# sasg/cilium

Hardware: AMD Instinct MI355X
Metric: classified headers/sec (Mpps, whole node) at 100k-prefix ipcache + 16k-ID policy (higher is better)
Workload: dtype u32

## Files before the change

cilium_amd/_lib.py:

```python
import ctypes
import os

HERE = os.path.dirname(os.path.abspath(__file__))
LIB_PATH = os.path.join(HERE, os.environ.get("CFC_LIB", "libcfc.so"))

CFC_DEVICE_NONE = -1
MODE_INGRESS, MODE_EGRESS, MODE_XDP, MODE_FULL = 0, 1, 2, 3
HF_FRAG, HF_TCP_CLOSE, HF_EXTHDR = 0x100, 0x200, 0x400
DROP_PREFILTER, VERDICT_PUNT = -1, -2
OPT_LPM4, OPT_TIMING, OPT_CT_APPLY, OPT_CT_EVICT = 1, 2, 3, 4
CT_APPLY_DEVICE, CT_APPLY_HOST = 0, 1
LPM4_AUTO, LPM4_DIR24_8, LPM4_TRIE = 0, 1, 2

EXPORTS = (
    "cfc_open", "cfc_close", "cfc_abi_version", "cfc_map_open",
    "cfc_drop_notify_v4", "cfc_drop_notify_v6",
    "cfc_map_close", "cfc_map_update", "cfc_map_lookup", "cfc_map_delete",
    "cfc_map_get_next_key", "cfc_num_possible_cpus", "cfc_endpoint_config",
    "cfc_commit", "cfc_classify_v4", "cfc_counters_device",
    "cfc_counters_sync", "cfc_counters_clear", "cfc_counters_export",
    "cfc_counters_import", "cfc_get_stats", "cfc_strerror",
    "cfc_set_option", "cfc_timing_collect", "cfc_classify_v6",
    "cfc_ct_apply_v4", "cfc_ct_apply_v6", "cfc_map_update_batch",
    "cfc_set_node_config", "cfc_get_node_config", "cfc_identity_counters",
    "cfc_set_clock", "cfc_monitor_events_v4", "cfc_monitor_events_v6",
    "cfc_map_dump", "cfc_ct_gc",
    "cfc_proxy_entries_v4", "cfc_proxy_entries_v6",
    "cfc_proxy_apply_v4", "cfc_proxy_apply_v6",
)
CT_NEW, CT_ESTABLISHED, CT_REPLY, CT_RELATED = 0, 1, 2, 3
CT_RES_MASK, CT_DONE, CT_CREATE = 0x3, 0x4, 0x8


class CfcError(OSError):
    pass


GC_REMOVE_EXPIRED, GC_VALID_IPS, GC_MATCH_IPS = 1, 2, 4


class Ip(ctypes.Structure):
    _fields_ = [("family", ctypes.c_uint8), ("pad", ctypes.c_uint8 * 3),
                ("addr", ctypes.c_uint8 * 16)]


class GcFilter(ctypes.Structure):
    _fields_ = [("flags", ctypes.c_uint32), ("time", ctypes.c_uint32),
                ("valid_ips", ctypes.c_void_p), ("n_valid", ctypes.c_uint32),
                ("pad0", ctypes.c_uint32),
                ("match_ips", ctypes.c_void_p), ("n_match", ctypes.c_uint32),
                ("pad1", ctypes.c_uint32)]


class GcStats(ctypes.Structure):
    _fields_ = [("deleted", ctypes.c_uint64), ("alive", ctypes.c_uint64),
                ("device_deleted", ctypes.c_uint64), ("log_deleted", ctypes.c_uint64),
                ("host_deleted", ctypes.c_uint64), ("slots_freed", ctypes.c_uint64)]


_HDR = [("saddr", ctypes.c_void_p), ("daddr", ctypes.c_void_p),
        ("ports", ctypes.c_void_p), ("meta", ctypes.c_void_p),
        ("mark", ctypes.c_void_p), ("tcp_flags", ctypes.c_void_p),
        ("n", ctypes.c_uint64)]


class HdrV4(ctypes.Structure):
    _fields_ = _HDR + [("hash", ctypes.c_void_p)]


class HdrV6(ctypes.Structure):
    _fields_ = _HDR + [("hash", ctypes.c_void_p)]


class Out(ctypes.Structure):
    _fields_ = [("verdict", ctypes.c_void_p), ("identity", ctypes.c_void_p),
                ("action", ctypes.c_void_p), ("ct", ctypes.c_void_p),
                ("notify", ctypes.c_void_p), ("pkt_saddr", ctypes.c_void_p),
                ("pkt_daddr", ctypes.c_void_p), ("pkt_ports", ctypes.c_void_p)]


class Stats(ctypes.Structure):
    _fields_ = [("epoch", ctypes.c_uint64), ("device_bytes", ctypes.c_uint64),
                ("ipcache_v4_prefixes", ctypes.c_uint32),
                ("lpm4_tbl8_groups", ctypes.c_uint32),
                ("policy_entries", ctypes.c_uint32),
                ("endpoints", ctypes.c_uint32),
                ("prefilter_v4_fix", ctypes.c_uint32),
                ("prefilter_v4_dyn", ctypes.c_uint32),
                ("lpm4_layout", ctypes.c_uint32),
                ("lpm4_kib", ctypes.c_uint32),
                ("ipcache_v6_prefixes", ctypes.c_uint32),
                ("lpm6_lengths", ctypes.c_uint32),
                ("lpm6_groups", ctypes.c_uint32),
                ("lpm6_kib", ctypes.c_uint32),
                ("endpoints_v6", ctypes.c_uint32),
                ("prefilter_v6_fix", ctypes.c_uint32),
                ("prefilter_v6_dyn", ctypes.c_uint32),
                ("ct4_entries", ctypes.c_uint32),
                ("ct6_entries", ctypes.c_uint32),
                ("ct_apply_device", ctypes.c_uint32),
                ("ct_apply_host", ctypes.c_uint32),
                ("ct_slots", ctypes.c_uint32),
                ("ct_grown", ctypes.c_uint32),
                ("ct_order_changed", ctypes.c_uint64),
                ("nat_hops", ctypes.c_uint64),
                ("ct_evicted", ctypes.c_uint64),
                ("svc_ordered", ctypes.c_uint64),
                ("ct_apply_sparse", ctypes.c_uint64),
                ("ct_self_segments", ctypes.c_uint64)]


class NodeConfig(ctypes.Structure):
    _fields_ = [("ipv4_cluster_range", ctypes.c_uint32),
                ("ipv4_cluster_mask", ctypes.c_uint32),
                ("router_ip6", ctypes.c_uint8 * 16),
                ("host_ifindex", ctypes.c_uint32)]


class IdentityCount(ctypes.Structure):
    _fields_ = [("identity", ctypes.c_uint32), ("dir", ctypes.c_uint8),
                ("pad", ctypes.c_uint8 * 3),
                ("fwd_packets", ctypes.c_uint64), ("fwd_bytes", ctypes.c_uint64),
                ("drop_packets", ctypes.c_uint64), ("drop_bytes", ctypes.c_uint64)]


IDENTITY_OUT_OF_RANGE = 0xFFFFFFFF


class ProxyStats(ctypes.Structure):
    _fields_ = [("redirects", ctypes.c_uint64), ("entries", ctypes.c_uint64),
                ("created", ctypes.c_uint64), ("updated", ctypes.c_uint64),
                ("failed", ctypes.c_uint64)]


class Timing(ctypes.Structure):
    _fields_ = [("launches", ctypes.c_uint64), ("classify_ms", ctypes.c_double),
                ("count_ms", ctypes.c_double), ("launches_v6", ctypes.c_uint64),
                ("classify_v6_ms", ctypes.c_double), ("count_v6_ms", ctypes.c_double)]


_lib = None


def lib():
    global _lib
    if _lib is not None:
        return _lib
    if not os.path.exists(LIB_PATH):
        raise CfcError(2, f"{LIB_PATH} is not built (run __graft_entry__.build())")
    L = ctypes.CDLL(LIB_PATH)
    vp, u32, u64, i32 = ctypes.c_void_p, ctypes.c_uint32, ctypes.c_uint64, ctypes.c_int
    pint = ctypes.POINTER(ctypes.c_int)
    L.cfc_open.argtypes = [i32, ctypes.POINTER(vp)]
    L.cfc_close.argtypes = [vp]
    L.cfc_close.restype = None
    L.cfc_map_open.argtypes = [vp, ctypes.c_char_p, u32, u32, u32, u32, u32,
                               pint, pint]
    L.cfc_map_close.argtypes = [vp, i32]
    L.cfc_map_update.argtypes = [vp, i32, vp, vp, u64]
    L.cfc_map_lookup.argtypes = [vp, i32, vp, vp]
    L.cfc_map_update_batch.argtypes = [vp, i32, vp, vp, u64, u64]
    L.cfc_map_delete.argtypes = [vp, i32, vp]
    L.cfc_map_get_next_key.argtypes = [vp, i32, vp, vp]
    L.cfc_map_dump.argtypes = [vp, i32, vp, vp, u64, ctypes.POINTER(u64)]
    L.cfc_endpoint_config.argtypes = [vp, ctypes.c_uint16, u32]
    L.cfc_set_node_config.argtypes = [vp, ctypes.POINTER(NodeConfig)]
    L.cfc_get_node_config.argtypes = [vp, ctypes.POINTER(NodeConfig)]
    L.cfc_commit.argtypes = [vp, vp]
    L.cfc_classify_v4.argtypes = [vp, ctypes.POINTER(HdrV4), ctypes.POINTER(Out),
                                  i32, ctypes.c_uint16, vp]
    L.cfc_classify_v6.argtypes = [vp, ctypes.POINTER(HdrV6), ctypes.POINTER(Out),
                                  i32, ctypes.c_uint16, vp]
    L.cfc_ct_apply_v4.argtypes = [vp, ctypes.POINTER(HdrV4), ctypes.POINTER(Out),
                                  i32, ctypes.c_uint16, vp]
    L.cfc_ct_apply_v6.argtypes = [vp, ctypes.POINTER(HdrV6), ctypes.POINTER(Out),
                                  i32, ctypes.c_uint16, vp]
    L.cfc_set_clock.argtypes = [vp, u32]
    L.cfc_ct_gc.argtypes = [vp, i32, ctypes.POINTER(GcFilter), ctypes.POINTER(GcStats), vp]
    for f in (L.cfc_drop_notify_v4, L.cfc_drop_notify_v6,
              L.cfc_monitor_events_v4, L.cfc_monitor_events_v6):
        f.argtypes = [vp, vp, ctypes.POINTER(Out), i32, ctypes.c_uint16, vp, vp,
                      u64, vp, vp]
    for f in (L.cfc_proxy_entries_v4, L.cfc_proxy_entries_v6):
        f.argtypes = [vp, vp, ctypes.POINTER(Out), i32, ctypes.c_uint16, vp, vp,
                      u64, vp, vp]
    for f in (L.cfc_proxy_apply_v4, L.cfc_proxy_apply_v6):
        f.argtypes = [vp, vp, ctypes.POINTER(Out), i32, ctypes.c_uint16,
                      ctypes.POINTER(ProxyStats), vp]
    L.cfc_counters_device.argtypes = [vp, ctypes.POINTER(vp), ctypes.POINTER(u64)]
    L.cfc_counters_sync.argtypes = [vp, vp]
    L.cfc_counters_clear.argtypes = [vp, vp]
    L.cfc_counters_export.argtypes = [vp, vp, u64, vp]
    L.cfc_counters_import.argtypes = [vp, vp, u64, vp]
    L.cfc_get_stats.argtypes = [vp, ctypes.POINTER(Stats)]
    L.cfc_identity_counters.argtypes = [vp, vp, u64, ctypes.POINTER(u64)]
    L.cfc_set_option.argtypes = [vp, i32, ctypes.c_int64]
    L.cfc_timing_collect.argtypes = [vp, ctypes.POINTER(Timing)]
    L.cfc_strerror.argtypes = [i32]
    L.cfc_strerror.restype = ctypes.c_char_p
    _lib = L
    return L


def check(rc, what):
    if rc < 0:
        raise CfcError(-rc, f"{what}: {os.strerror(-rc)}")
    return rc
```

cilium_amd/csrc/cfc_api.cpp:

```cpp
#include <hip/hip_runtime.h>

#include <algorithm>
#include <cerrno>
#include <cstdio>
#include <cstdlib>
#include <cstring>
#include <map>
#include <set>
#include <memory>
#include <mutex>
#include <string>
#include <thread>
#include <unordered_set>
#include <type_traits>
#include <vector>

#include "../../include/cfc.h"
#include "classify.hpp"
#include "selfcut.hpp"
#include "ctmirror.hpp"
#include "flatten.hpp"
#include "maps.hpp"

using namespace cfc;

namespace {

template <class T>
static int upload_vec(DevBuf &b, const std::vector<T> &v, hipStream_t s)
{
    return b.upload(v.data(), v.size() * sizeof(T), s);
}

struct GIpc {
    DevBuf tbl24, tbl8, ovf, l4d, l4c, l4l;
    int layout = 0;
    uint32_t n_prefix4 = 0, tbl8_groups = 0, lpm4_kib = 0;
    uint64_t bytes = 0;
};
struct GIpc6 {
    DevBuf l6[4];
    Lpm6 ipc6{};
    Lpm6Host host;
    uint32_t lpm6_kib = 0, n_prefix6 = 0, lpm6_lengths = 0, lpm6_groups = 0;
    uint64_t bytes = 0;
};
struct GPf {
    DevBuf pf24, pf8, pffix, pfbloom, pf6bloom, l6fix[4], l6dyn[4];
    Lpm6 fix{}, dyn{};
    uint32_t fix_mask = 0, fix_zero = 0, bloom_words = 0, bloom6_words = 0;
    uint32_t n_fix4 = 0, n_dyn4 = 0, n_fix6 = 0, n_dyn6 = 0;
    uint64_t bytes = 0;
};
struct GEp {
    DevBuf lxc4, lxc6, pol, polbloom;
    std::vector<PolSlot> pol_host;
    uint32_t lxc4_mask = 0, lxc6_mask = 0, pol_bloom_words = 0, n_eps = 0, n_eps6 = 0;
    bool lxc4_lds = false, lxc6_lds = false;
    std::unordered_map<int, PolLoc> pol_loc;
    std::vector<std::pair<Map *, std::string>> ctr_owner;
    std::vector<uint32_t> seclabel;
    DevBuf ep_info;
    std::map<uint16_t, uint32_t> nat4;
    DevBuf nat6;
    uint64_t bytes = 0;
};
struct GLb {
    DevBuf lb4, rnat4, lb6, rnat6;
    uint32_t lb4_mask = 0, n_lb4 = 0, lb6_mask = 0, n_lb6 = 0;
    uint64_t bytes = 0;
};
struct GCt {
    CtTab<Ct4Slot> t4;
    CtTab<Ct6Slot> t6;
    DevBuf ct_sum;
    DevBuf ct_st;
    CtMaps ct_maps;
    uint32_t n_nat46 = 0;
    uint64_t bytes = 0;
};
template <bool V6, class G>
auto &tab(G &g)
{
    if constexpr (V6)
        return g.t6;
    else
        return g.t4;
}
template <bool V6>
uint64_t state_base(const GCt &g)
{
    return V6 ? g.t4.slots : 0;
}
struct Epoch {
    uint64_t id = 0;
    std::shared_ptr<GIpc> ipc;
    std::shared_ptr<GIpc6> ipc6;
    std::shared_ptr<GPf> pf;
    std::shared_ptr<GEp> ep;
    std::shared_ptr<GCt> ct;
    std::shared_ptr<GLb> lb;
    DevTables T{};
    cfc_stats st{};
};
struct Retired {
    std::shared_ptr<Epoch> e;
    std::vector<hipEvent_t> ev;
};

}

struct cfc_ctx {
    int device = 0;
    int num_cus = 256;
    std::recursive_mutex mu;
    std::map<std::string, std::unique_ptr<Map>> maps;
    std::map<int, Map *> fds;
    int next_fd = 3;
    std::vector<uint32_t> seclabel = std::vector<uint32_t>(65536, 0);
// ... 47 lines not shown
    DevBuf ord_delbm, ord_mixbm, ord_dfirst, ord_cnt;
    DevBuf ord_ct0;
    DevBuf cta_mon;
    uint64_t n_ord_changed = 0;
    struct NatRec {
        int family = 0;
        const void *saddr = nullptr;
        uint64_t n = 0;
        int mode = 0;
        uint16_t ep = 0;
        uint32_t m = 0;
        hipStream_t stream = nullptr;
        DevBuf idx, rows, outs, ws;
        cfc_hdr_v4 h4{};
        cfc_hdr_v6 h6{};
        cfc_out o{};
    };
    std::map<const void *, NatRec> nat;
    DevBuf nat_list, nat_cnt, nat_tmp;
    DevBuf svo_keys, svo_keys2, svo, svo_cnt, svo_tmp;
    uint64_t n_apply_sparse = 0;
    bool nat46_seen = false, hop_nat46 = false;
    uint64_t n_nat_hops = 0;
    bool ct_evict = true;
    DevBuf evict_bm, evict_maps, evict_rel;
    uint64_t n_evicted = 0;
    uint64_t n_ct_grow = 0;
    DevBuf self_addr, self_rows, self_cnt;
    uint64_t n_self_segs = 0;
    struct SegRec {
        const void *saddr = nullptr;
        uint64_t n = 0, off = 0;
        int mode = 0, family = 0;
        uint16_t ep = 0;
    };
    std::map<const void *, SegRec> segs;
    bool pend = false, pend_v6 = false;
    uint32_t *pend_cnt = nullptr;
    hipEvent_t pend_ev = nullptr;
    DevBuf cta_cxr;

    uint64_t *ctr = nullptr;
    size_t ctr_u64 = 0;
    bool ctr_pending = false;
    hipStream_t last_stream = nullptr;
    hipEvent_t last_done = nullptr;
    uint32_t *ws = nullptr;
    size_t ws_bytes = 0;
    Map *metrics = nullptr;
    std::vector<uint64_t> idc = std::vector<uint64_t>(ID_U64, 0);

    DevBuf nt_ws;
    hipEvent_t nt_done = nullptr;
    hipStream_t nt_stream = nullptr;
    bool nt_pending = false;

    DevBuf px_cnt, px_own, px_last, px_bm, px_blk, px_rec;
    hipEvent_t px_done = nullptr;
    hipStream_t px_stream = nullptr;
    bool px_pending = false;

    bool timing = false;
    std::vector<LaunchTiming> tpool;
    size_t tused = 0;
};

namespace {

void order_after_launches(cfc_ctx *c, hipStream_t s)
{
    if (c->ctr_pending && c->last_done && c->last_stream != s)
        (void)hipStreamWaitEvent(s, c->last_done, 0);
    if (c->nt_pending && c->nt_done && c->nt_stream != s)
        (void)hipStreamWaitEvent(s, c->nt_done, 0);
}

constexpr int NGROUPS = 6;
void group_sigs(cfc_ctx *c, uint64_t sig[NGROUPS])
{
    for (int g = 0; g < NGROUPS; g++)
        sig[g] = 1469598103934665603ull + (uint64_t)g;
    auto mix = [&](int g, uint64_t v) { sig[g] = (sig[g] ^ v) * 1099511628211ull; };
    mix(0, (uint64_t)c->opts.lpm4);
    mix(2, c->seclabel_gen);
    for (auto &kv : c->maps) {
        const Map *m = kv.second.get();
        const uint64_t id = (uint64_t)(uintptr_t)m;
        switch (m->role) {
        case ROLE_IPCACHE:
            mix(0, id); mix(0, m->sgen[0]);
            mix(4, id); mix(4, m->sgen[1]);
            break;
        case ROLE_PF4_FIX: case ROLE_PF4_DYN: case ROLE_PF6_FIX: case ROLE_PF6_DYN:
            mix(1, id); mix(1, m->sgen[0]);
            break;
        case ROLE_LXC:
            mix(2, id); mix(2, m->gen);
            break;
        case ROLE_POLICY:
            mix(2, id); mix(2, m->sgen[0]);
            break;
        case ROLE_CT4: case ROLE_CT6:
            mix(3, id); mix(3, m->sgen[0]);
            mix(2, id);
            break;
        case ROLE_LB4_SVC: case ROLE_LB4_RNAT: case ROLE_LB6_SVC: case ROLE_LB6_RNAT:
            mix(5, id); mix(5, m->gen);
            mix(3, m->kv.empty() ? 0 : 1);
            break;
        default:
            break;
        }
    }
}

void settle(cfc_ctx *c)
{
    if (!c->pend)
        return;
    c->pend = false;
    (void)hipEventSynchronize(c->pend_ev);
    const uint32_t *h = c->pend_cnt;
    cfc_ctx::CtFam &X = c->ctf[c->pend_v6];
    X.claims += h[CTA_CLAIMS];
    X.ins += h[CTA_CLAIMS];
    X.log_used += h[CTA_NLOG];
}

template <class Slot>
int remap_mirror(CtTab<Slot> &T, hipStream_t s)
{
    std::vector<Slot> &h = T.host;
    DevBuf &pend = T.pend;
    if (!pend.p)
        return 0;
    const uint64_t n = h.size();
    std::vector<uint32_t> map(n);
    if (n && (hipMemcpyAsync(map.data(), pend.p, 4 * n, hipMemcpyDeviceToHost, s) != hipSuccess ||
              hipStreamSynchronize(s) != hipSuccess))
        return -EIO;
    std::vector<Slot> nh(T.slots);
    const unsigned nt = std::max(1u, std::min(16u, std::thread::hardware_concurrency()));
    std::vector<uint64_t> tb(nt, 0);
    std::vector<std::thread> th;
    for (unsigned t = 0; t < nt; t++)
        th.emplace_back([&, t]() {
            for (uint64_t i = n * t / nt, e = n * (t + 1) / nt; i < e; i++)
                if (map[i] != 0xFFFFFFFFu) {
                    nh[map[i]] = h[i];
                    tb[t] += h[i].w == CT_TOMBSTONE;
                }
        });
    for (std::thread &x : th)
        x.join();
    uint64_t tt = 0;
    for (uint64_t v : tb)
        tt += v;
    T.tomb = (uint32_t)tt;
    h.swap(nh);
    pend.reset();
    return 0;
}
int mirror_sync(GCt &G, hipStream_t s)
{
    if (int rc = remap_mirror(G.t4, s))
        return rc;
// ... 185 lines not shown
            v[1] += byt;
            if (it == mm->kv.end() && mm->kv.size() >= mm->max_entries)
                continue;
            Map::Entry &e = mm->kv[nk];
            e.key = nk;
            e.val.assign((const char *)v, 16);
            mm->gen++;
        }
    c->ctr_pending = false;
    return 0;
}

int upload_lpm6(DevBuf *b, const Lpm6Host &h, Lpm6 *d, hipStream_t s)
{
    int rc;
    if ((rc = upload_vec(b[0], h.slots, s)) || (rc = upload_vec(b[1], h.bloom, s)) ||
        (rc = upload_vec(b[2], h.lens, s)) || (rc = upload_vec(b[3], h.slots64, s)))
        return rc;
    d->slots = (const L6Slot *)b[0].p;
    d->slots64 = (const uint4 *)b[3].p;
    d->mask64 = h.slots64.empty() ? 0 : (uint32_t)h.slots64.size() - 1;
    d->bloom = (const uint64_t *)b[1].p;
    d->lens = (const uint32_t *)b[2].p;
    d->mask = h.slots.empty() ? 0 : (uint32_t)h.slots.size() - 1;
    d->bloom_mask = h.bloom.empty() ? 0 : (uint32_t)h.bloom.size() - 1;
    d->nlen = (uint32_t)h.lens.size();
    d->def_label = h.def_label;
    return 0;
}

void note_stream(cfc_ctx *c, hipStream_t s)
{
    if (std::find(c->streams.begin(), c->streams.end(), s) == c->streams.end())
        c->streams.push_back(s);
}

uint32_t identity_cover_touched(cfc_ctx *c)
{
    uint32_t cover = 0;
    for (auto &kv : c->maps) {
        Map *m = kv.second.get();
        if (m->role != ROLE_IPCACHE)
            continue;
        for (auto &t : m->touched) {
            auto it = m->kv.find(t.first);
            if (it == m->kv.end())
                continue;
            uint32_t lab;
            memcpy(&lab, it->second.val.data(), 4);
            if (lab < ID_PACK_LIMIT)
                cover |= 1u << id_range_of(lab);
        }
    }
    return cover;
}

void reap_retired(cfc_ctx *c)
{
    auto done = [](const Retired &r) {
        for (hipEvent_t e : r.ev)
            if (hipEventQuery(e) != hipSuccess)
                return false;
        return true;
    };
    for (size_t i = 0; i < c->retired.size();) {
        if (done(c->retired[i])) {
            for (hipEvent_t e : c->retired[i].ev)
                (void)hipEventDestroy(e);
            c->retired.erase(c->retired.begin() + (long)i);
        } else {
            i++;
        }
    }
}

std::shared_ptr<GIpc> build_ipc(const HostImage &img, hipStream_t s, int *rc)
{
    auto g = std::make_shared<GIpc>();
    if ((*rc = upload_vec(g->tbl24, img.tbl24, s)) || (*rc = upload_vec(g->tbl8, img.tbl8, s)) ||
        (*rc = upload_vec(g->ovf, img.lbl_ovf, s)) || (*rc = upload_vec(g->l4d, img.l4d, s)) ||
        (*rc = upload_vec(g->l4c, img.l4c, s)) || (*rc = upload_vec(g->l4l, img.l4l, s)))
        return nullptr;
    g->layout = img.lpm4_layout;
    g->n_prefix4 = img.n_prefix4;
    g->tbl8_groups = (uint32_t)(img.tbl8.size() / 256);
    g->lpm4_kib = (uint32_t)((4ull * (img.l4d.size() + img.l4c.size() + img.tbl24.size() +
                                      img.tbl8.size()) + 8ull * img.l4l.size() + 1023) / 1024);
    g->bytes = 4ull * (img.tbl24.size() + img.tbl8.size() + img.lbl_ovf.size() +
                       img.l4d.size() + img.l4c.size()) + 8ull * img.l4l.size();
    return g;
}

std::shared_ptr<GIpc6> build_ipc6(HostImage &img, hipStream_t s, int *rc)
{
    auto g = std::make_shared<GIpc6>();
    if ((*rc = upload_lpm6(g->l6, img.ipc6, &g->ipc6, s)))
        return nullptr;
    g->n_prefix6 = img.ipc6.n;
    g->lpm6_lengths = (uint32_t)img.ipc6.lens.size();
    g->lpm6_groups = img.ipc6.groups;
    g->lpm6_kib = (uint32_t)((img.ipc6.bytes() + 1023) / 1024);
    g->bytes = img.ipc6.bytes();
    g->host = std::move(img.ipc6);
    return g;
}

uint32_t identity_cover(const std::vector<Map *> &ms)
{
    uint32_t cover = 1u;
    for (Map *m : ms)
        if (m->role == ROLE_IPCACHE)
            for (const auto &kv : m->kv) {
                uint32_t lab;
                memcpy(&lab, kv.second.val.data(), 4);
                if (lab < ID_PACK_LIMIT)
                    cover |= 1u << id_range_of(lab);
            }
    return cover;
}

std::shared_ptr<GPf> build_pf(const HostImage &img, hipStream_t s, int *rc)
{
    auto g = std::make_shared<GPf>();
    if ((*rc = upload_vec(g->pf24, img.pf_tbl24, s)) || (*rc = upload_vec(g->pf8, img.pf_tbl8, s)) ||
        (*rc = upload_vec(g->pffix, img.pf_fix, s)) ||
        (*rc = upload_vec(g->pfbloom, img.pf_bloom, s)) ||
        (*rc = upload_vec(g->pf6bloom, img.pf6_bloom, s)) ||
        (*rc = upload_lpm6(g->l6fix, img.pf6_fix, &g->fix, s)) ||
        (*rc = upload_lpm6(g->l6dyn, img.pf6_dyn, &g->dyn, s)))
        return nullptr;
    g->fix_mask = img.pf_fix_mask;
    g->fix_zero = img.pf_fix_zero;
    g->bloom_words = (uint32_t)img.pf_bloom.size();
    g->bloom6_words = (uint32_t)img.pf6_bloom.size();
    g->n_fix4 = img.n_pf_fix;
    g->n_dyn4 = img.n_pf_dyn;
    g->n_fix6 = img.pf6_fix.n;
    g->n_dyn6 = img.pf6_dyn.n;
    g->bytes = 4ull * (img.pf_tbl24.size() + img.pf_tbl8.size() + img.pf_fix.size() +
                       img.pf_bloom.size() + img.pf6_bloom.size()) + img.pf6_fix.bytes() +
               img.pf6_dyn.bytes();
    return g;
}

std::shared_ptr<GEp> build_ep(cfc_ctx *c, HostImage &img, const std::vector<Map *> &ms,
                              hipStream_t s, int *rc)
{
    auto g = std::make_shared<GEp>();
    if ((*rc = upload_vec(g->lxc4, img.lxc4, s)) || (*rc = upload_vec(g->pol, img.pol, s)) ||
        (*rc = upload_vec(g->polbloom, img.pol_bloom, s)) ||
        (*rc = upload_vec(g->lxc6, img.lxc6, s)))
        return nullptr;
    g->lxc4_mask = img.lxc4_mask;
    g->lxc6_mask = img.lxc6_mask;
    g->lxc4_lds = img.lxc4.size() <= LXC_LDS_MAX_SLOTS;
    g->lxc6_lds = img.lxc6.size() <= LXC6_LDS_MAX_SLOTS;
    g->pol_bloom_words = (uint32_t)img.pol_bloom.size();
    g->pol_host = img.pol;
    g->n_eps = img.n_eps;
    g->n_eps6 = img.n_eps6;
    g->pol_loc = std::move(img.pol_loc);
    g->ctr_owner = std::move(img.ctr_owner);
    g->bytes = sizeof(LxcSlot) * img.lxc4.size() + sizeof(PolSlot) * img.pol.size() +
               4ull * img.pol_bloom.size() + sizeof(Lxc6Slot) * img.lxc6.size();
    g->seclabel = c->seclabel;
    std::vector<uint2> info(65536, make_uint2(0, 0));
// ... 28 lines not shown
    auto g = std::make_shared<GLb>();
    if ((*rc = upload_vec(g->lb4, img.lb4, s)) || (*rc = upload_vec(g->rnat4, img.rnat4, s)) ||
        (*rc = upload_vec(g->lb6, img.lb6, s)) || (*rc = upload_vec(g->rnat6, img.rnat6, s)))
        return nullptr;
    g->lb4_mask = img.lb4_mask;
    g->n_lb4 = img.n_lb4;
    g->lb6_mask = img.lb6_mask;
    g->n_lb6 = img.n_lb6;
    g->bytes = 16ull * img.lb4.size() + 8ull * img.rnat4.size() + 16ull * img.lb6.size() +
               16ull * img.rnat6.size();
    return g;
}

std::shared_ptr<GCt> build_ctg(HostImage &img, const std::vector<Map *> &ms, hipStream_t s,
                               int *rc)
{
    auto g = std::make_shared<GCt>();
    if ((*rc = upload_vec(g->t4.key, img.ct4, s)) || (*rc = upload_vec(g->t6.key, img.ct6, s)) ||
        (*rc = upload_vec(g->t4.lb, img.ct4_lb, s)) || (*rc = upload_vec(g->t6.lb, img.ct6_lb, s)))
        return nullptr;
    const size_t nslots = img.ct4.size() + img.ct6.size();
    if (nslots && (*rc = g->ct_sum.zeros(4 * nslots, s)))
        return nullptr;
    const size_t n4 = img.ct4.size(), n6 = img.ct6.size();
    if (nslots) {
        DevBuf tm;
        if (g->ct_st.ensure(sizeof(CtState) * nslots) ||
            tm.ensure(sizeof(CtTimer) * std::max(n4, n6))) {
            *rc = -ENOMEM;
            return nullptr;
        }
        g->ct_st.bytes = sizeof(CtState) * nslots;
        CtState *st = (CtState *)g->ct_st.p;
        for (int f = 0; f < 2; f++) {
            const std::vector<CtTimer> &v = f ? img.ct6_tm : img.ct4_tm;
            if (v.empty())
                continue;
            if (hipMemcpyAsync(tm.p, v.data(), sizeof(CtTimer) * v.size(),
                               hipMemcpyHostToDevice, s) != hipSuccess ||
                ct_state_init(st + (f ? n4 : 0), (const CtTimer *)tm.p, v.size(), s) ||
                hipStreamSynchronize(s) != hipSuccess) {
                *rc = -EIO;
                return nullptr;
            }
        }
    }
    if (n4 && (*rc = g->t4.ms.zeros(12 * n4, s)))
        return nullptr;
    if (n6 && (*rc = g->t6.ms.zeros(12 * n6, s)))
        return nullptr;
    for (Map *m : ms)
        if (m->role == ROLE_CT4 || m->role == ROLE_CT6)
            g->ct_maps[ct_map_key(m->role == ROLE_CT4 ? 4 : 6,
                                  ct_owner_word((uint32_t)std::max(m->policy_lxc, 0),
                                                m->policy_lxc >= 0),
                                  m->ct_any)] = m;
    g->t4.mask = img.ct4_mask;
    g->t4.probe = img.ct4_probe;
    g->t6.mask = img.ct6_mask;
    g->t6.probe = img.ct6_probe;
    g->t4.n = img.n_ct4;
    g->t6.n = img.n_ct6;
    g->n_nat46 = img.n_nat46;
    g->bytes = sizeof(Ct4Slot) * img.ct4.size() + sizeof(Ct6Slot) * img.ct6.size() +
               (sizeof(CtState) + 4) * nslots + 8ull * (n4 + n6) + 16ull * img.ct4_lb.size();
    g->t4.slots = img.ct4.size();
    g->t6.slots = img.ct6.size();
    g->t4.host = std::move(img.ct4);
    g->t6.host = std::move(img.ct6);
    return g;
}

void assemble(Epoch &E)
{
    DevTables &T = E.T;
    T = DevTables{};
    const GIpc &I = *E.ipc;
    const GIpc6 &I6 = *E.ipc6;
    const GPf &P = *E.pf;
    const GEp &D = *E.ep;
    const GCt &C = *E.ct;
    const GLb &B = *E.lb;
    T.l4d = (const uint4 *)I.l4d.p;
    T.l4c = (const uint32_t *)I.l4c.p;
    T.l4l = (const uint64_t *)I.l4l.p;
    T.tbl24 = (const uint32_t *)I.tbl24.p;
    T.tbl8 = (const uint32_t *)I.tbl8.p;
    T.lbl_ovf = (const uint32_t *)I.ovf.p;
    T.ipc6 = I6.ipc6;
    T.pf_tbl24 = (const uint32_t *)P.pf24.p;
    T.pf_tbl8 = (const uint32_t *)P.pf8.p;
    T.pf_fix = (const uint32_t *)P.pffix.p;
    T.pf_fix_mask = P.fix_mask;
    T.pf_fix_zero = P.fix_zero;
    T.pf_bloom = (const uint32_t *)P.pfbloom.p;
    T.pf_bloom_words = P.bloom_words;
    T.pf6_fix = P.fix;
    T.pf6_bloom = (const uint32_t *)P.pf6bloom.p;
    T.pf6_bloom_words = P.bloom6_words;
    T.pf6_dyn = P.dyn;
    T.lxc4 = (const LxcSlot *)D.lxc4.p;
    T.lxc4_mask = D.lxc4_mask;
    T.lxc4_lds = D.lxc4_lds;
    T.lxc6 = (const Lxc6Slot *)D.lxc6.p;
    T.lxc6_mask = D.lxc6_mask;
    T.lxc6_lds = D.lxc6_lds;
    T.pol = (const PolSlot *)D.pol.p;
    T.pol_bloom = (const uint32_t *)D.polbloom.p;
    T.pol_bloom_words = D.pol_bloom_words;
    T.n_ctr = (uint32_t)D.ctr_owner.size();
    T.ct4 = (C.t4.n || C.t4.slots) ? (const Ct4Slot *)C.t4.key.p : nullptr;
    T.ct6 = (C.t6.n || C.t6.slots) ? (const Ct6Slot *)C.t6.key.p : nullptr;
    T.ct_st = (CtState *)C.ct_st.p;
    T.ct_sum = (uint32_t *)C.ct_sum.p;
    T.ct4_mask = C.t4.mask;
    T.ct4_probe = C.t4.mask;
    T.ct6_mask = C.t6.mask;
    T.ct6_probe = C.t6.mask;
    T.ct6_acct_base = (uint32_t)state_base<true>(C);
    T.lb4 = B.n_lb4 ? (const uint4 *)B.lb4.p : nullptr;
    T.lb4_mask = B.lb4_mask;
    T.rnat4 = (const uint2 *)B.rnat4.p;
    T.ct4_lb = T.ct4 ? (const uint4 *)C.t4.lb.p : nullptr;
    T.lb6 = B.n_lb6 ? (const uint4 *)B.lb6.p : nullptr;
    T.lb6_mask = B.lb6_mask;
    T.rnat6 = (const uint4 *)B.rnat6.p;
    T.ct6_lb = T.ct6 ? (const uint4 *)C.t6.lb.p : nullptr;
    cfc_stats &st = E.st;
    st = cfc_stats{};
    st.epoch = E.id;
    st.device_bytes = I.bytes + I6.bytes + P.bytes + D.bytes + C.bytes + B.bytes;
    st.ipcache_v4_prefixes = I.n_prefix4;
    st.lpm4_tbl8_groups = I.tbl8_groups;
    st.policy_entries = T.n_ctr;
    st.endpoints = D.n_eps;
    st.prefilter_v4_fix = P.n_fix4;
    st.prefilter_v4_dyn = P.n_dyn4;
    st.lpm4_layout = (uint32_t)I.layout;
    st.lpm4_kib = I.lpm4_kib;
    st.ipcache_v6_prefixes = I6.n_prefix6;
    st.lpm6_lengths = I6.lpm6_lengths;
    st.lpm6_groups = I6.lpm6_groups;
    st.lpm6_kib = I6.lpm6_kib;
    st.endpoints_v6 = D.n_eps6;
    st.prefilter_v6_fix = P.n_fix6;
    st.prefilter_v6_dyn = P.n_dyn6;
    st.ct4_entries = C.t4.n;
    st.ct6_entries = C.t6.n;
}

bool patch_ct(cfc_ctx *c, hipStream_t s);

unsigned patch_touched(cfc_ctx *c, unsigned groups, hipStream_t s)
{
    Epoch &E = *c->epoch;
    for (auto &kv : c->maps) {
        Map *m = kv.second.get();
        if (m->touched.empty())
            continue;
        if (m->role == ROLE_IPCACHE) {
            for (auto &t : m->touched) {
                auto it = m->kv.find(t.first);
                if (it == m->kv.end())
                    continue;
                const bool v6 = t.first.size() > 7 && (uint8_t)t.first[7] == 2;
                if (!v6) {
// ... 381 lines not shown

int cfc_abi_version(void) { return CFC_ABI_VERSION; }
int cfc_num_possible_cpus(void) { return 1; }

int cfc_open(int device, cfc_ctx **out)
{
    if (!out)
        return -EINVAL;
    if (device != CFC_DEVICE_NONE) {
        int ndev = 0;
        if (hipGetDeviceCount(&ndev) != hipSuccess || ndev <= 0)
            return -ENODEV;
        if (device < 0 || device >= ndev)
            return -ENODEV;
        if (hipSetDevice(device) != hipSuccess)
            return -ENODEV;
    }
    auto *c = new cfc_ctx();
    c->device = device;
    if (device != CFC_DEVICE_NONE) {
        hipDeviceProp_t p;
        if (hipGetDeviceProperties(&p, device) == hipSuccess &&
            p.multiProcessorCount > 0)
            c->num_cus = p.multiProcessorCount;
        (void)hipEventCreateWithFlags(&c->last_done, hipEventDisableTiming);
        (void)hipEventCreateWithFlags(&c->nt_done, hipEventDisableTiming);
        (void)hipEventCreateWithFlags(&c->px_done, hipEventDisableTiming);
    }
    auto m = std::make_unique<Map>();
    m->name = "cilium_metrics";
    m->role = ROLE_METRICS;
    m->type = MT_PERCPU_HASH;
    m->ksz = 8;
    m->vsz = 16;
    m->max_entries = 65536;
    c->metrics = m.get();
    c->maps["cilium_metrics"] = std::move(m);
    *out = c;
    return 0;
}

void cfc_close(cfc_ctx *c)
{
    if (!c)
        return;
    if (c->device != CFC_DEVICE_NONE) {
        (void)hipSetDevice(c->device);
        (void)hipDeviceSynchronize();
    }
    for (Retired &r : c->retired)
        for (hipEvent_t e : r.ev)
            (void)hipEventDestroy(e);
    c->retired.clear();
    c->epoch.reset();
    free_timing(c);
    if (c->ctr)
        (void)hipFree(c->ctr);
    if (c->ws)
        (void)hipFree(c->ws);
    if (c->last_done)
        (void)hipEventDestroy(c->last_done);
    if (c->pend_ev)
        (void)hipEventDestroy(c->pend_ev);
    if (c->pend_cnt)
        (void)hipHostFree(c->pend_cnt);
    if (c->nt_done)
        (void)hipEventDestroy(c->nt_done);
    if (c->px_done)
        (void)hipEventDestroy(c->px_done);
    delete c;
}

int cfc_set_option(cfc_ctx *c, int option, int64_t value)
{
    if (!c)
        return -EINVAL;
    std::lock_guard<std::recursive_mutex> g(c->mu);
    switch (option) {
    case CFC_OPT_LPM4:
        if (value < CFC_LPM4_AUTO || value > CFC_LPM4_TRIE)
            return -EINVAL;
        c->opts.lpm4 = (int)value;
        return 0;
    case CFC_OPT_TIMING:
        if (value != 0 && value != 1)
            return -EINVAL;
        if (c->device == CFC_DEVICE_NONE)
            return -ENODEV;
        c->timing = value != 0;
        return 0;
    case CFC_OPT_CT_APPLY:
        if (value != CFC_CT_APPLY_DEVICE && value != CFC_CT_APPLY_HOST)
            return -EINVAL;
        c->ct_apply_mode = (int)value;
        return 0;
    case CFC_OPT_CT_EVICT:
        if (value != 0 && value != 1)
            return -EINVAL;
        c->ct_evict = value != 0;
        return 0;
    default:
        return -EINVAL;
    }
}

int cfc_timing_collect(cfc_ctx *c, cfc_timing *out)
{
    if (!c || !out)
        return -EINVAL;
    std::lock_guard<std::recursive_mutex> g(c->mu);
    if (c->device == CFC_DEVICE_NONE)
        return -ENODEV;
    memset(out, 0, sizeof(*out));
    for (size_t i = 0; i < c->tused; i++) {
        const LaunchTiming &t = c->tpool[i];
        float a = 0, b = 0;
        if (hipEventSynchronize(t.ev[2]) != hipSuccess ||
            hipEventElapsedTime(&a, t.ev[0], t.ev[1]) != hipSuccess ||
            hipEventElapsedTime(&b, t.ev[1], t.ev[2]) != hipSuccess)
            return -EIO;
        out->launches++;
        out->classify_ms += a;
        out->count_ms += b;
        if (t.v6) {
            out->launches_v6++;
            out->classify_v6_ms += a;
            out->count_v6_ms += b;
        }
    }
    c->tused = 0;
    return 0;
}

int cfc_map_open(cfc_ctx *c, const char *path, uint32_t type, uint32_t ks,
                 uint32_t vs, uint32_t max_entries, uint32_t flags, int *fd,
                 int *created)
{
    if (!c || !path || !fd)
        return -EINVAL;
    if (type != MT_HASH && type != MT_PERCPU_HASH && type != MT_LRU_HASH &&
        type != MT_LPM_TRIE)
        return -EINVAL;
    if (!ks || !vs || !max_entries || (type == MT_LPM_TRIE && ks <= 4))
        return -EINVAL;
    std::lock_guard<std::recursive_mutex> g(c->mu);
    std::string p(path);
    std::string base = p.substr(p.find_last_of('/') + 1);
    int lxc = -1, ct_any = 0;
    Role r = role_for(p, &lxc, &ct_any);
    if (!role_geometry_ok(r, type, ks, vs))
        return -EINVAL;
    std::string key = r == ROLE_NONE ? p : base;
    auto it = c->maps.find(key);
    int was_created = 0;
    Map *m;
    if (it != c->maps.end()) {
        m = it->second.get();
        if (m->type != type || m->ksz != ks || m->vsz != vs ||
            (m->role != ROLE_METRICS && m->max_entries != max_entries))
            return -EINVAL;
    } else {
        auto nm = std::make_unique<Map>();
        nm->name = key;
        nm->role = r;
        nm->policy_lxc = lxc;
        nm->ct_any = ct_any;
        nm->type = type;
        nm->ksz = ks;
        nm->vsz = vs;
        nm->max_entries = max_entries;
        nm->flags = flags;
        m = nm.get();
        c->maps[key] = std::move(nm);
        was_created = 1;
    }
    *fd = c->next_fd++;
    c->fds[*fd] = m;
    if (created)
        *created = was_created;
    return 0;
}

int cfc_map_close(cfc_ctx *c, int fd)
{
    if (!c)
        return -EINVAL;
// ... 2813 lines not shown
```

cilium_amd/csrc/classify.hip:

```cpp
#include <algorithm>
#include <cstdlib>
#include <mutex>
#include <set>
#include <tuple>
#include <vector>

#include "kern_common.hpp"
#ifndef CFC_EXP
#define CFC_EXP 0
#endif

namespace cfc {

namespace {

constexpr int LDS_MET_U64 = 18;
template <int MODE>
constexpr int met_n()
{
    return MODE == CFC_MODE_EGRESS ? 7 : MODE == CFC_MODE_XDP ? 0 : 4;
}
template <int MODE>
constexpr int acc_n()
{
// ... 48 lines not shown
    int ct_res;
    uint32_t idw;
    bool id_ovf, drop1;
    bool nat;
    uint32_t ev2;
    uint32_t tf;
    uint32_t evw;
    uint32_t tda, tpt, psa, ppt, lbfl;
    PolicyProbe P;
};

struct Raw {
    uint32_t sa, da, pt, mt, mk, tf;
    uint32_t tda, tpt, psa, lbfl;
};
template <bool OPT, bool LBE>
__device__ __forceinline__ void r1_issue(const cfc_hdr_v4 &in, const LbIn &L, uint32_t i,
                                         uint32_t nloc, Raw &r)
{
    i = i < nloc ? i : nloc - 1;
#if CFC_EXP == 8
    i &= 8191;
#endif
    const uint32_t o = i << 2;
    r.sa = ldo_nt(in.saddr, o);
    r.da = ldo_nt(in.daddr, o);
    r.pt = ldo_nt(in.ports, o);
    r.mt = ldo_nt(in.meta, o);
    r.mk = r.tf = 0;
    if (OPT) {
        const uint32_t mk = ldo_nt(in.mark ? in.mark : in.saddr, o);
        const uint32_t tf = *((in.tcp_flags ? in.tcp_flags : (const uint8_t *)in.saddr) + i);
        r.mk = in.mark ? mk : 0u;
        r.tf = in.tcp_flags ? tf : 0u;
    }
    if (LBE) {
        r.tda = ldo_nt(L.tda, o);
        r.tpt = ldo_nt(L.tpt, o);
        r.psa = ldo_nt(L.psa, o);
        r.lbfl = ldo_nt(L.fl, o);
    } else {
        r.tda = r.da;
        r.tpt = r.pt;
        r.psa = r.sa;
        r.lbfl = 0;
    }
}
__device__ __forceinline__ void r1_take(const Raw &r, uint32_t i, uint32_t end,
                                        Hdr &h)
{
    h.valid = i < end;
    h.sa = r.sa;
    h.da = r.da;
    h.pt = r.pt;
    h.mt = r.mt;
    h.mk = r.mk;
    h.tf = r.tf;
    h.tda = r.tda;
    h.tpt = r.tpt;
    h.psa = r.psa;
    h.ppt = r.pt;
    h.lbfl = r.lbfl;
}

template <int MODE>
__device__ __forceinline__ void r2_issue(const DevTables &T, const Lds &S,
                                         Hdr &h)
{
    constexpr bool XDP = MODE == CFC_MODE_XDP || MODE == CFC_MODE_FULL;
    constexpr bool EGR = MODE == CFC_MODE_EGRESS;
    constexpr bool LPM = MODE != CFC_MODE_XDP;
    h.l4d = make_uint4(0, 0, 0, 0);
    h.e24 = h.pfd = 0;
    h.lx = h.ls = h.pf = make_uint4(0, 0, 0, 0);
    h.lh = __builtin_bswap32(EGR ? h.tda : h.sa);
    h.hsh = __builtin_bswap32(h.sa);
    h.lxs = h.lss = h.pfb = 0;
    h.pf_maybe = false;
    if (LPM) {
        if (T.l4d)
#if CFC_EXP == 1
            h.l4d = make_uint4(h.lh & 0xFFFF, 0, 0, 0);
#else
            h.l4d = ldt16(T.l4d, (h.lh >> 16) * 16u);
#endif
        else if (T.tbl24)
            h.e24 = T.tbl24[h.lh >> 8];
    }
    if (XDP && T.pf_tbl24)
        h.pfd = T.pf_tbl24[h.hsh >> 8];
    if (T.lxc4) {
        h.lxs = hash32(h.da, T.lxc4_mask);
        h.lx = lxc_slot(T, S, h.lxs);
        if (EGR) {
            h.lss = hash32(h.sa, T.lxc4_mask);
            h.ls = lxc_slot(T, S, h.lss);
        }
    }
    if (XDP && T.pf_fix && h.sa) {
        h.pf_maybe = !S.pfb || bloom_maybe(S.pfb_off, S.pfb_mask, pf_bloom_hash(h.sa));
        if (h.pf_maybe) {
            h.pfb = hash32(h.sa, T.pf_fix_mask);
            h.pf = ldt16(T.pf_fix, h.pfb * 16u);
        }
    }
}

template <int MODE, bool CT, bool LB>
__device__ __forceinline__ void r3_identity(const DevTables &T, const Lds &S,
                                            const EgressArgs &E, Hdr &h)
{
    constexpr bool XDP = MODE == CFC_MODE_XDP || MODE == CFC_MODE_FULL;
    constexpr bool EGR = MODE == CFC_MODE_EGRESS;
    constexpr bool LPM = MODE != CFC_MODE_XDP;
    if (LPM && T.l4d) {
#if CFC_EXP == 4
        h.e24 = (h.l4d.x & L4_PTR) ? 300u : h.l4d.x;
#else
        h.e24 = l4_lookup(T, h.lh, h.l4d);
#endif
    } else {
        if (h.e24 & LPM_GROUP)
            h.e24 = T.tbl8[((h.e24 & ~LPM_GROUP) << 8) | (h.lh & 0xFF)];
        if (h.e24 & LPM_INDIRECT)
            h.e24 = T.lbl_ovf[h.e24 & LPM_PAYLOAD];
    }
    if (h.pfd & LPM_GROUP)
        h.pfd = T.pf_tbl8[((h.pfd & ~LPM_GROUP) << 8) | (h.hsh & 0xFF)];
    h.rec = make_uint4(0, 0, 0, 0);
    uint4 srec = h.rec;
    if (T.lxc4) {
#if CFC_EXP == 7
        h.rec = h.lx;
#else
        h.rec = lxc_resolve(T, S, h.da, h.lxs, h.lx);
#endif
        if (EGR)
            srec = lxc_resolve(T, S, h.sa, h.lss, h.ls);
    }
    const bool local = (h.rec.w & LXC_VALID) != 0;
    h.src_lxc = (srec.w & LXC_VALID) ? (srec.w & 0xFFFF) : NONE;

    h.act = TC_ACT_OK;
    h.ver = 0;
    h.ident = 0;
    h.met0 = h.met1 = h.ctr0 = h.ctr1 = NONE;
    h.xdp_drop = false;
    if (XDP) {
        bool deny = h.pfd != 0;
        if (!deny)
            deny = h.sa ? (h.pf_maybe && pf_resolve(T, h.sa, h.pfb, h.pf))
                        : T.pf_fix_zero != 0;
        h.xdp_drop = deny || !local;
        if (MODE == CFC_MODE_XDP || h.xdp_drop) {
            h.act = h.xdp_drop ? XDP_DROP : XDP_PASS;
            h.ver = h.xdp_drop ? CFC_DROP_PREFILTER : 0;
        }
    }

    h.need_pol = h.skip_proxy = false;
    h.pbase = h.pmask = h.egress_bit = h.dport = 0;
    h.ct_byte = 0;
    h.ct_slot = NONE;
    h.ct_res = CT_NEW;
    h.ct_k1 = h.ct_k2 = NONE;
    h.idw = KEY_NONE;
    h.id_ovf = h.drop1 = false;
// ... 219 lines not shown
                                                        E.seclabel, dp2, proto,
                                                        0, frag);
            const int w = pw.verdict;
            ctr1 = pw.ctr;
            if (CT)
                ctb |= ((uint32_t)c2.res | CTO_DONE |
                        ((c2.res == CT_NEW && (w >= 0 || reply2)) ? CTO_CREATE : 0u)) << 4;
            if (hop) {
                nat = true;
                act = TC_ACT_OK;
                ver = 0;
            } else if (w < 0 && !reply2) {
                act = TC_ACT_SHOT;
                ver = DROP_POLICY;
                met1 = mkey<MODE>(DROP_POLICY, METRIC_INGRESS);
                ev2 = 2;
            } else {
                const bool prox = w > 0 && !reply2;
                act = (prox || ifx) ? TC_ACT_REDIRECT : TC_ACT_OK;
                ver = prox ? w : 0;
                met1 = prox ? NONE : mkey<MODE>(0, METRIC_INGRESS);
                ev2 = 1;
                if (NT) {
                    uint32_t mon2 = ct_monitor(T, CT ? T.ct_st : nullptr,
                                               CT ? c2.slot : NONE, CT_INGRESS,
                                               action, tfl, dp2);
                    if (fresh)
                        mon2 = dp2 == 0x3500u ? MTU_LEN
                               : ct_monitor_of(T, make_uint4(0, T.now, 0, 0), CT_INGRESS,
                                               action, tfl);
                    evw = trace_word(prox ? OBS_TO_PROXY : OBS_TO_LXC, h.rec.w & 0xFFFF,
                                     CT ? (uint32_t)c2.res : 0u, mon2);
                }
            }
        }
    }
    h.ev2 = ev2;
    if (EGR)
        h.nat = nat;
    h.evw = evw;
    h.act = act;
    h.ver = ver;
    h.met0 = met0;
    h.met1 = met1;
    h.ctr0 = pr.ctr;
    h.ctr1 = ctr1;
    h.ct_byte = ctb;
}

struct LdsPlan {
    uint32_t lxc_slots, pf_words, pol_words;
    __host__ __device__ size_t bytes() const
    {
        return 8ull * LDS_MET_U64 + 16ull * lxc_slots + 4ull * pf_words +
               4ull * pol_words;
    }
};

__host__ LdsPlan lds_plan(const DevTables &T)
{
    LdsPlan p;
    p.lxc_slots = (T.lxc4 && T.lxc4_lds) ? T.lxc4_mask + 1 : 0;
    p.pf_words = T.pf_bloom ? T.pf_bloom_words : 0;
    p.pol_words = T.pol_bloom ? T.pol_bloom_words : 0;
    return p;
}

template <int MODE>
__device__ __forceinline__ void acc_publish(const unsigned long long *s_met,
                                            const CountArgs &C, uint32_t seclabel)
{
    for (uint32_t j = threadIdx.x; j < 2u * acc_n<MODE>(); j += BLOCK) {
        const unsigned long long v = s_met[j];
        if (!v)
            continue;
        const uint32_t k = j >> 1;
        uint64_t *dst = k < (uint32_t)met_n<MODE>()
                            ? C.g_met + met_reason_dir<MODE>(k) * 2
                            : C.g_id + id_index(ID_DIR_INGRESS, seclabel, k - met_n<MODE>());
        atomicAdd((unsigned long long *)dst + (j & 1), v);
    }
}

template <int MODE, int U, bool CT, bool NT, bool OPT, bool LB, bool FAST>
__global__ __launch_bounds__(BLOCK, WAVES_PER_SIMD) void k_classify_v4(
    DevTables T, LdsPlan L, cfc_hdr_v4 in, cfc_out out, EgressArgs E,
    CountArgs C, uint64_t per_block, LbIn LI)
{
    if (FAST) {
        T.tbl24 = T.tbl8 = T.pf_tbl24 = T.pf_tbl8 = nullptr;
        __builtin_assume(T.l4d != nullptr);
        __builtin_assume(T.lxc4 != nullptr);
        if (MODE == CFC_MODE_XDP || MODE == CFC_MODE_FULL)
            __builtin_assume(T.pf_fix != nullptr);
    }
    unsigned long long *s_met = lds_met();
    Lds S;
    S.lxc_off = LDS_MET_U64 / 2;
    const uint32_t pf4 = S.lxc_off + L.lxc_slots;
    const uint32_t pol4 = pf4 + L.pf_words / 4;
    S.pfb_off = 4 * pf4;
    S.polb_off = 4 * pol4;
    S.lxc = FAST || L.lxc_slots != 0;
    S.pfb = FAST || L.pf_words != 0;
    S.polb = FAST || L.pol_words != 0;
    S.pfb_mask = L.pf_words - 1;
    S.polb_mask = L.pol_words - 1;
    for (uint32_t j = threadIdx.x; j < (uint32_t)LDS_MET_U64; j += BLOCK)
        s_met[j] = 0;
    constexpr bool WL = CT && MODE != CFC_MODE_XDP && !LB;
    lds_copy(cfc_smem + S.lxc_off, reinterpret_cast<const uint4 *>(T.lxc4),
             L.lxc_slots);
    lds_copy(cfc_smem + pf4, reinterpret_cast<const uint4 *>(T.pf_bloom),
             L.pf_words / 4);
    lds_copy(cfc_smem + pol4, reinterpret_cast<const uint4 *>(T.pol_bloom),
             L.pol_words / 4);
    __syncthreads();

    constexpr bool EGR = MODE == CFC_MODE_EGRESS;
    const uint32_t id_dir = EGR ? ID_DIR_EGRESS : ID_DIR_INGRESS;
    const uint64_t start = (uint64_t)blockIdx.x * per_block;
    if (start >= in.n)
        return;
    const uint32_t end = (uint32_t)min(in.n - start, per_block);
    in.saddr += start;
    in.daddr += start;
    in.ports += start;
    in.meta += start;
    if (OPT) {
        if (in.mark)
            in.mark += start;
        if (in.tcp_flags)
            in.tcp_flags += start;
        if (out.action)
            out.action += start;
        if (out.ct)
            out.ct += start;
    }
    out.verdict += start;
    out.identity += start;
    if (out.notify)
        out.notify += start;
    constexpr bool LBE = LB && MODE == CFC_MODE_EGRESS;
    if (LBE) {
        LI.tda += start;
        LI.tpt += start;
        LI.psa += start;
        LI.fl += start;
    }
    if (LB && out.pkt_saddr) {
        out.pkt_saddr += start;
        out.pkt_daddr += start;
        out.pkt_ports += start;
    }
    if (C.ct)
        C.ct += start;
    if (C.ct2)
        C.ct2 += start;
    if (C.ctr)
        C.ctr += start;
    if (C.ctr2)
        C.ctr2 += start;
    if (C.id)
        C.id += start;
    MetAcc<acc_n<MODE>()> acc;
    acc.clear();
    uint32_t iter = 0;
    Raw nx[U];
#pragma unroll
    for (int u = 0; u < U; u++)
        r1_issue<OPT, LBE>(in, LI, u * BLOCK + threadIdx.x, end, nx[u]);
    for (uint32_t base = 0; base < end; base += BLOCK * U) {
        Hdr h[U];
// ... 797 lines not shown
    __shared__ uint32_t tmp[32];
    const uint64_t b0 = (uint64_t)blockIdx.x * 4 * BLOCK + 4ull * threadIdx.x;
    uint32_t v[4], s = 0;
#pragma unroll
    for (int j = 0; j < 4; j++) {
        v[j] = b0 + j < n ? in[b0 + j] : 0u;
        s += v[j];
    }
    uint32_t e = block_excl_scan(s, tmp);
#pragma unroll
    for (int j = 0; j < 4; j++) {
        if (b0 + j < n)
            out[b0 + j] = e;
        e += v[j];
    }
    if (threadIdx.x == BLOCK - 1)
        bsum[blockIdx.x] = e;
}
__global__ __launch_bounds__(BLOCK) void k_scan_top(uint32_t *bsum, uint32_t nb,
                                                    uint32_t *total)
{
    __shared__ uint32_t tmp[32];
    uint32_t carry = 0;
    for (uint32_t c = 0; c < nb; c += BLOCK) {
        const uint32_t i = c + threadIdx.x;
        const uint32_t v = i < nb ? bsum[i] : 0u;
        const uint32_t e = block_excl_scan(v, tmp);
        if (i < nb)
            bsum[i] = carry + e;
        carry += tmp[31];
        __syncthreads();
    }
    if (threadIdx.x == 0)
        *total = carry;
}
__global__ __launch_bounds__(BLOCK) void k_scan_add(uint32_t *out, uint64_t n,
                                                    const uint32_t *bsum)
{
    const uint64_t b0 = (uint64_t)blockIdx.x * 4 * BLOCK + 4ull * threadIdx.x;
    const uint32_t add = bsum[blockIdx.x];
#pragma unroll
    for (int j = 0; j < 4; j++)
        if (b0 + j < n)
            out[b0 + j] += add;
}

__global__ __launch_bounds__(256) void k_add_u64(uint64_t *dst,
                                                 const uint64_t *src,
                                                 uint64_t n)
{
    uint64_t i = (uint64_t)blockIdx.x * 256 + threadIdx.x;
    if (i < n)
        dst[i] += src[i];
}

__global__ __launch_bounds__(256) void k_patch16(const Patch16 *rec, uint64_t n)
{
    const uint64_t i = (uint64_t)blockIdx.x * 256 + threadIdx.x;
    if (i < n) {
        const uint4 v = *(const uint4 *)rec[i].val;
        *(uint4 *)rec[i].dst = v;
    }
}

#ifndef CFC_FAST
#define CFC_FAST 1
#endif
bool fast_shape(const DevTables &T, int mode, const LdsPlan &L)
{
    if (!CFC_FAST)
        return false;
    const bool xdp = mode == CFC_MODE_XDP || mode == CFC_MODE_FULL;
    return T.l4d && !T.tbl24 && !T.pf_tbl24 && T.lxc4 && L.lxc_slots && L.pol_words &&
           (!xdp || (T.pf_fix && L.pf_words));
}

template <int MODE, bool CT, bool NT>
void launch_mode_nt(const DevTables &T, const cfc_hdr_v4 &in, const cfc_out &out,
                    const EgressArgs &E, const CountArgs &C, uint32_t grid,
                    uint64_t per_block, hipStream_t s, const LbIn *lb)
{
    const LdsPlan L = lds_plan(T);
    const bool opt = in.mark || in.tcp_flags || out.action || (CT && out.ct);
    const bool fast = fast_shape(T, MODE, L);
    auto kern = opt ? (fast ? k_classify_v4<MODE, CFC_UNROLL, CT, NT, true, false, true>
                            : k_classify_v4<MODE, CFC_UNROLL, CT, NT, true, false, false>)
                    : (fast ? k_classify_v4<MODE, CFC_UNROLL, CT, NT, false, false, true>
                            : k_classify_v4<MODE, CFC_UNROLL, CT, NT, false, false, false>);
    const LbIn none{};
    if constexpr (CT && MODE != CFC_MODE_XDP) {
        if (lb)
            kern = k_classify_v4<MODE, CFC_UNROLL, CT, NT, true, true, false>;
    }
    set_lds_limit((const void *)kern, (int)LDS_PER_WG);
    hipLaunchKernelGGL(kern, dim3(grid), dim3(BLOCK), L.bytes(), s, T, L, in,
                       out, E, C, per_block, lb ? *lb : none);
}

template <int MODE, bool CT>
void launch_mode(const DevTables &T, const cfc_hdr_v4 &in, const cfc_out &out,
                 const EgressArgs &E, const CountArgs &C, uint32_t grid,
                 uint64_t per_block, hipStream_t s, const LbIn *lb)
{
    if (out.notify)
        launch_mode_nt<MODE, CT, true>(T, in, out, E, C, grid, per_block, s, lb);
    else
        launch_mode_nt<MODE, CT, false>(T, in, out, E, C, grid, per_block, s, lb);
}

uint32_t hist_slices(uint64_t n, uint64_t slots)
{
    if (!n || !slots)
        return 0;
    uint64_t nb = std::min<uint64_t>(256, (n + 4095) / 4096);
    nb = std::min<uint64_t>(nb, std::max<uint64_t>(1, (256ull << 20) / (4 * slots)));
    nb = std::max<uint64_t>(nb, (n + SLICE_MAX - 1) / SLICE_MAX);
    return (uint32_t)std::max<uint64_t>(nb, 1);
}

uint64_t hist_per_block(uint64_t n, uint32_t nblk)
{
    const uint64_t pb = (n + nblk - 1) / nblk;
    return (pb + 3) & ~3ull;
}

uint64_t hist_slots(const DevTables &T, int mode)
{
    if (mode == CFC_MODE_XDP)
        return 0;
    uint64_t id_slots = 0;
    for (uint32_t r = 0; r < ID_RANGES; r++)
        if ((T.id_cover >> r) & 1)
            id_slots += std::min<uint64_t>(2 * ID_RANGE, 2ull * ID_PACK_LIMIT - 2ull * r * ID_RANGE);
    return (mode == CFC_MODE_EGRESS ? 2ull : 1ull) * T.n_ctr + id_slots;
}

}

void set_lds_limit(const void *kernel, int bytes)
{
    static std::mutex mu;
    static std::set<std::tuple<int, const void *, int>> done;
    int dev = 0;
    (void)hipGetDevice(&dev);
    std::lock_guard<std::mutex> g(mu);
    if (done.insert(std::make_tuple(dev, kernel, bytes)).second)
        (void)hipFuncSetAttribute(kernel, hipFuncAttributeMaxDynamicSharedMemorySize,
                                  bytes);
}

size_t classify_lds_bytes(const DevTables &T) { return lds_plan(T).bytes(); }

int launch_patch16(const Patch16 *rec, uint64_t n, hipStream_t s)
{
    if (!n)
        return 0;
    hipLaunchKernelGGL(k_patch16, dim3((unsigned)((n + 255) / 256)), dim3(256), 0, s, rec, n);
    return hipGetLastError() == hipSuccess ? 0 : -5;
}

int launch_add_u64(uint64_t *dst, const uint64_t *src, uint64_t n,
                   hipStream_t s)
{
    if (!n)
        return 0;
    hipLaunchKernelGGL(k_add_u64, dim3((unsigned)((n + 255) / 256)), dim3(256),
                       0, s, dst, src, n);
    return hipGetLastError() == hipSuccess ? 0 : -5;
}

uint32_t ctp_buckets(const DevTables &T)
{
    if (getenv("CFC_ACC_PER_SLICE"))
        return 0;
    const uint64_t slots = (T.ct4 ? T.ct4_mask + 1ull : 0) + (T.ct6 ? T.ct6_mask + 1ull : 0);
// ... 254 lines not shown
```

cilium_amd/csrc/flatten.cpp:

```cpp
#include "flatten.hpp"

#include <algorithm>
#include <cstring>
#include <map>

namespace cfc {

static constexpr uint64_t POL_SLOTS_PER_KEY = 4;
static uint32_t pow2_at_least(uint64_t x)
{
    uint32_t p = 1;
    while (p < x)
        p <<= 1;
    return p;
}

uint64_t HostImage::device_bytes() const
{
    return 4ull * (tbl24.size() + tbl8.size() + lbl_ovf.size() +
                   pf_tbl24.size() + pf_tbl8.size() + pf_fix.size() +
                   pf_bloom.size() + pol_bloom.size()) +
           4ull * (l4d.size() + l4c.size()) + 8ull * l4l.size() +
           sizeof(LxcSlot) * lxc4.size() + sizeof(PolSlot) * pol.size() +
           ipc6.bytes() + pf6_fix.bytes() + pf6_dyn.bytes() +
           sizeof(Lxc6Slot) * lxc6.size() + sizeof(Ct4Slot) * ct4.size() +
           sizeof(Ct6Slot) * ct6.size() + 48ull * (ct4.size() + ct6.size());
}

void build_dir24_8(std::vector<Pfx4> pfx, std::vector<uint32_t> *tbl24,
                   std::vector<uint32_t> *tbl8)
{
    std::stable_sort(pfx.begin(), pfx.end(),
                     [](const Pfx4 &a, const Pfx4 &b) { return a.plen < b.plen; });
    tbl24->assign(1u << 24, 0);
    tbl8->clear();
    uint32_t *t24 = tbl24->data();
    for (const Pfx4 &p : pfx) {
        if (p.plen > 24)
            break;
        uint32_t start = p.plen ? (p.addr >> 8) & ~((1u << (24 - p.plen)) - 1) : 0;
        std::fill(t24 + start, t24 + start + (1u << (24 - p.plen)), p.leaf);
    }
    for (const Pfx4 &p : pfx) {
        if (p.plen <= 24)
            continue;
        uint32_t idx = p.addr >> 8;
        if (!(t24[idx] & LPM_GROUP)) {
            uint32_t g = (uint32_t)(tbl8->size() >> 8);
            tbl8->resize(tbl8->size() + 256, t24[idx]);
            t24[idx] = LPM_GROUP | g;
        }
        uint32_t g = t24[idx] & ~LPM_GROUP;
        uint32_t lo = p.addr & 0xFF & ~((1u << (32 - p.plen)) - 1);
        uint32_t *grp = tbl8->data() + ((size_t)g << 8);
        std::fill(grp + lo, grp + lo + (1u << (32 - p.plen)), p.leaf);
    }
}

namespace {

struct L4Trie {
    std::vector<uint32_t> *d, *c, *ovf;
    std::vector<uint64_t> *l;
    bool ok = true;

    uint32_t list_leaf(uint32_t leaf)
    {
        if (leaf & LPM_INDIRECT)
            return LL_INDIRECT | (leaf & LPM_PAYLOAD);
        if (leaf > LL_PAYLOAD) {
            ovf->push_back(leaf);
            return LL_INDIRECT | (uint32_t)(ovf->size() - 1);
        }
        return leaf;
    }
    uint64_t entry(uint32_t addr, int len, uint32_t leaf)
    {
        return ((uint64_t)(((uint32_t)len & 31) << 27 | list_leaf(leaf)) << 32) | addr;
    }

    uint32_t node(std::vector<Pfx4> &longp, uint32_t base, int lvl, uint32_t def,
                  uint32_t *dir = nullptr)
    {
        if (longp.empty())
            return def;
        if (longp.size() + 1 < L4_LIST_MAX) {
            std::stable_sort(longp.begin(), longp.end(),
                             [](const Pfx4 &a, const Pfx4 &b) { return a.plen > b.plen; });
            size_t first = 0;
            if (dir) {
                uint64_t e[L4_INLINE] = {0, 0};
                for (; first < longp.size() && first < L4_INLINE; first++)
                    e[first] = l4_inline_entry(longp[first].addr, longp[first].plen,
                                               list_leaf(longp[first].leaf));
                dir[1] = (uint32_t)e[0];
                dir[2] = (uint32_t)(e[0] >> 32) | (uint32_t)(e[1] << 16);
                dir[3] = (uint32_t)(e[1] >> 16);
                if (first == longp.size())
                    return def;
            }
            const size_t off = l->size();
            for (size_t i = first; i < longp.size(); i++)
                l->push_back(entry(longp[i].addr, longp[i].plen, longp[i].leaf));
            l->push_back(entry(base, lvl, def));
            if (l->size() & 1)
                l->push_back(l->back());
            if (off > L4_OFF)
                ok = false;
            return L4_PTR | (uint32_t)(l->size() - off) << 24 | (uint32_t)(off & L4_OFF);
        }
        const int nl = lvl + 8;
        const uint32_t sh = 32 - nl;
        const size_t off = c->size();
        c->resize(off + 256, 0);
        uint32_t defs[256];
        std::fill(defs, defs + 256, def);
        std::vector<std::vector<Pfx4>> sub(256);
        std::stable_sort(longp.begin(), longp.end(),
                         [](const Pfx4 &a, const Pfx4 &b) { return a.plen < b.plen; });
        for (const Pfx4 &p : longp) {
            const uint32_t j = (p.addr >> sh) & 255;
            if (p.plen <= nl) {
                const uint32_t span = 1u << (nl - p.plen);
                std::fill(defs + (j & ~(span - 1)), defs + (j & ~(span - 1)) + span, p.leaf);
            } else {
                sub[j].push_back(p);
            }
        }
        for (uint32_t j = 0; j < 256; j++) {
            const uint32_t e = node(sub[j], base | (j << sh), nl, defs[j]);
            (*c)[off + j] = e;
        }
        if (off > L4_OFF)
            ok = false;
        return L4_PTR | (uint32_t)off;
    }
};

}

bool build_l4trie(std::vector<Pfx4> pfx, std::vector<uint32_t> *ovf,
                  std::vector<uint32_t> *l4d, std::vector<uint32_t> *l4c,
                  std::vector<uint64_t> *l4l)
{
    std::stable_sort(pfx.begin(), pfx.end(),
                     [](const Pfx4 &a, const Pfx4 &b) { return a.plen < b.plen; });
    l4d->assign(4u << 16, 0);
    l4c->clear();
    l4l->clear();
    for (const Pfx4 &p : pfx) {
        if (p.plen > 16)
            break;
        const uint32_t start = p.plen ? (p.addr >> 16) & ~((1u << (16 - p.plen)) - 1) : 0;
        for (uint32_t j = start; j < start + (1u << (16 - p.plen)); j++)
            (*l4d)[4 * j] = p.leaf;
    }
    std::map<uint32_t, std::vector<Pfx4>> by16;
    for (const Pfx4 &p : pfx)
        if (p.plen > 16)
            by16[p.addr >> 16].push_back(p);
    L4Trie b{l4d, l4c, ovf, l4l};
    for (auto &g : by16) {
        uint32_t *dir = l4d->data() + 4 * g.first;
        dir[0] = b.node(g.second, g.first << 16, 16, dir[0], dir);
    }
    return b.ok;
}

namespace {

typedef std::pair<uint64_t, uint64_t> U128;

U128 masked128(const uint32_t w[4], uint32_t len)
{
    uint32_t m[4];
    for (int i = 0; i < 4; i++)
        m[i] = w[i] & l6_word_mask(len, i);
    return {(uint64_t)m[0] << 32 | m[1], (uint64_t)m[2] << 32 | m[3]};
}

size_t max_pile(const std::vector<std::vector<const Pfx6 *>> &by_len,
                const std::vector<uint32_t> &L, size_t i, size_t k)
{
    std::vector<U128> v;
    for (size_t j = i; j <= k; j++)
        for (const Pfx6 *p : by_len[L[j]])
            v.push_back(masked128(p->w, L[k]));
    std::sort(v.begin(), v.end());
    size_t best = 0;
    for (size_t a = 0; a < v.size();) {
        size_t b = a;
        while (b < v.size() && v[b] == v[a])
            b++;
        best = std::max(best, b - a);
        a = b;
    }
    return best;
}

}

void build_lpm6(const std::vector<Pfx6> &pfx, Lpm6Host *out)
{
    *out = Lpm6Host();
    out->n = (uint32_t)pfx.size();
    std::vector<std::vector<const Pfx6 *>> by_len(129);
    size_t nkeys = 0;
    for (const Pfx6 &p : pfx) {
        if (p.plen == 0) {
            out->def_label = p.label;
        } else {
            by_len[p.plen].push_back(&p);
            nkeys++;
        }
    }
    std::vector<uint32_t> L;
    for (uint32_t l = 128; l >= 1; l--)
        if (!by_len[l].empty())
            L.push_back(l);
    if (L.empty())
        return;
    uint32_t sel_of[129] = {0};
    for (size_t i = 0; i < L.size();) {
        size_t k = i;
        while (k + 1 < L.size() && max_pile(by_len, L, i, k + 1) <= L6_GROUP_MAX)
            k++;
        for (size_t j = i; j <= k; j++) {
            out->lens.push_back(L[j] | L[k] << 8 | (j == i ? L6_GROUP_FIRST : 0));
            sel_of[L[j]] = L[k];
        }
        out->groups++;
        i = k + 1;
    }
    out->bloom.assign(pow2_at_least(std::max<size_t>(64, nkeys / 4)), 0);
    const uint32_t bmask = (uint32_t)out->bloom.size() - 1;
    size_t n64 = 0;
    for (uint32_t len : L)
        n64 += len <= 64 ? by_len[len].size() : 0;
    if (nkeys > n64)
        out->slots.assign(pow2_at_least(std::max<size_t>(16, 2 * (nkeys - n64))), L6Slot{});
    if (n64)
        out->slots64.assign(pow2_at_least(std::max<size_t>(16, 2 * n64)), make_uint4(0, 0, 0, 0));
    const uint32_t ns = (uint32_t)out->slots.size(), ns64 = (uint32_t)out->slots64.size();
    for (uint32_t len : L)
        for (const Pfx6 *p : by_len[len]) {
            const uint32_t h = l6_hash(p->w[0], p->w[1], p->w[2], p->w[3], len);
            out->bloom[l6_group_hash(p->w, sel_of[len]) & bmask] |= l6_bloom_bits(h);
            if (len <= 64) {
                uint32_t s = h & (ns64 - 1);
// ... 24 lines not shown
        uint32_t m[4];
        for (int i = 0; i < 4; i++)
            m[i] = w[i] & l6_word_mask(len, i);
        const uint32_t h = l6_hash(m[0], m[1], m[2], m[3], len);
        const uint64_t b = l6_bloom_bits(h);
        if ((bw & b) != b)
            continue;
        if (len <= 64) {
            const uint32_t mask64 = (uint32_t)t.slots64.size() - 1;
            for (uint32_t s = h & mask64;; s = (s + 1) & mask64) {
                const uint4 &d = t.slots64[s];
                if (!d.w)
                    break;
                if (d.w == len && d.x == m[0] && d.y == m[1])
                    return d.z;
            }
            continue;
        }
        for (uint32_t s = h & mask;; s = (s + 1) & mask) {
            const L6Slot &d = t.slots[s];
            if (!d.len)
                break;
            if (d.len == len && !memcmp(d.w, m, 16))
                return d.label;
        }
    }
    return t.def_label;
}

static void bloom_size(std::vector<uint32_t> *b, size_t keys, uint32_t max_words)
{
    uint32_t w = pow2_at_least(std::max<size_t>(64, keys));
    b->assign(std::min(w, max_words), 0u);
}
static inline void bloom_add(std::vector<uint32_t> *b, uint32_t h)
{
    (*b)[h & (b->size() - 1)] |= bloom_bits(h);
}

static uint32_t leaf_for(uint32_t label, std::vector<uint32_t> *ovf)
{
    if (label < LPM_INDIRECT)
        return label;
    ovf->push_back(label);
    return LPM_INDIRECT | (uint32_t)(ovf->size() - 1);
}

static inline uint32_t bswap(uint32_t x) { return __builtin_bswap32(x); }

static void ipcache_v4(const Map *m, std::vector<Pfx4> *out,
                       std::vector<uint32_t> *ovf)
{
    static const uint8_t stat4[4] = {0, 0, 0, 1};
    std::map<std::pair<uint32_t, int>, std::pair<uint32_t, uint32_t>> best;
    for (const auto &kv : m->kv) {
        const uint8_t *k = (const uint8_t *)kv.first.data();
        uint32_t P;
        memcpy(&P, k, 4);
        if (P > 64)
            continue;
        bool ok = true;
        for (uint32_t bit = 0; bit < std::min<uint32_t>(P, 32); bit++) {
            uint32_t byte = bit >> 3, sh = 7 - (bit & 7);
            if (((k[4 + byte] >> sh) & 1) != ((stat4[byte] >> sh) & 1)) {
                ok = false;
                break;
            }
        }
        if (!ok)
            continue;
        int plen = P > 32 ? (int)(P - 32) : 0;
        uint32_t a;
        memcpy(&a, k + 8, 4);
        uint32_t label;
        memcpy(&label, kv.second.val.data(), 4);
        auto key = std::make_pair(bswap(a), plen);
        auto it = best.find(key);
        if (it == best.end() || it->second.first < P)
            best[key] = {P, label};
    }
    for (const auto &b : best)
        out->push_back({b.first.first, (uint8_t)b.first.second,
                        leaf_for(b.second.second, ovf)});
}

bool ipcache_v6_entry(const std::string &nk, const std::string &val, Pfx6 *p)
{
    static const uint8_t stat6[4] = {0, 0, 0, 2};
    const uint8_t *k = (const uint8_t *)nk.data();
    uint32_t P;
    memcpy(&P, k, 4);
    if (P <= 32 || P > 160 || nk.size() < 24 || val.size() < 4)
        return false;
    for (uint32_t bit = 0; bit < 32; bit++) {
        uint32_t byte = bit >> 3, sh = 7 - (bit & 7);
        if (((k[4 + byte] >> sh) & 1) != ((stat6[byte] >> sh) & 1))
            return false;
    }
    p->plen = (uint8_t)(P - 32);
    for (int i = 0; i < 4; i++) {
        uint32_t a;
        memcpy(&a, k + 8 + 4 * i, 4);
        p->w[i] = bswap(a) & l6_word_mask(p->plen, i);
    }
    memcpy(&p->label, val.data(), 4);
    return true;
}

int64_t lpm6_find_slot(const Lpm6Host &t, const Pfx6 &p)
{
    if (p.plen && p.plen <= 64) {
        if (t.slots64.empty())
            return -1;
        const uint32_t mask = (uint32_t)t.slots64.size() - 1;
        uint32_t s = l6_hash(p.w[0], p.w[1], p.w[2], p.w[3], p.plen) & mask;
        for (uint32_t n = 0; n <= mask; n++, s = (s + 1) & mask) {
            const uint4 &d = t.slots64[s];
            if (!d.w)
                return -1;
            if (d.w == p.plen && d.x == p.w[0] && d.y == p.w[1])
                return L6_S64 | s;
        }
        return -1;
    }
    if (t.slots.empty() || !p.plen)
        return -1;
    const uint32_t mask = (uint32_t)t.slots.size() - 1;
    uint32_t s = l6_hash(p.w[0], p.w[1], p.w[2], p.w[3], p.plen) & mask;
    for (uint32_t n = 0; n <= mask; n++, s = (s + 1) & mask) {
        const L6Slot &d = t.slots[s];
        if (!d.len)
            return -1;
        if (d.len == p.plen && !memcmp(d.w, p.w, 16))
            return s;
    }
    return -1;
}

static void ipcache_v6(const Map *m, std::vector<Pfx6> *out)
{
    static const uint8_t stat6[4] = {0, 0, 0, 2};
    std::map<std::pair<U128, int>, std::pair<uint32_t, Pfx6>> best;
    for (const auto &kv : m->kv) {
        const uint8_t *k = (const uint8_t *)kv.first.data();
        uint32_t P;
        memcpy(&P, k, 4);
        if (P > 160)
            continue;
        bool ok = true;
        for (uint32_t bit = 0; bit < std::min<uint32_t>(P, 32); bit++) {
            uint32_t byte = bit >> 3, sh = 7 - (bit & 7);
            if (((k[4 + byte] >> sh) & 1) != ((stat6[byte] >> sh) & 1)) {
                ok = false;
                break;
            }
        }
        if (!ok)
            continue;
        Pfx6 p;
        p.plen = (uint8_t)(P > 32 ? P - 32 : 0);
        for (int i = 0; i < 4; i++) {
            uint32_t a;
            memcpy(&a, k + 8 + 4 * i, 4);
            p.w[i] = bswap(a) & l6_word_mask(p.plen, i);
        }
        memcpy(&p.label, kv.second.val.data(), 4);
// ... 257 lines not shown
                img->ct6[i] = e;
                img->ct6_tm[i] = tm;
                if (!img->ct6_lb.empty()) {
                    const uint4 l = ct_lb_of(kv.second.val);
                    img->ct6_lb[i] = make_uint4(l.x & 0xFFFF, l.y, 0, 0);
                }
                img->ct6_probe = std::max(img->ct6_probe, p);
                img->n_ct6++;
            }
            if (m->policy_lxc >= 0)
                img->ct_local[m->policy_lxc] = 1;
        }
        if (m->policy_lxc >= 0)
            img->ct_local[m->policy_lxc] = 1;
    }
}

void build_image(const std::vector<Map *> &maps, const BuildOpts &opt,
                 HostImage *img, unsigned groups)
{
    const uint64_t ct_min4 = img->ct_min4, ct_min6 = img->ct_min6;
    *img = HostImage();
    img->ct_min4 = ct_min4;
    img->ct_min6 = ct_min6;
    img->ct_local.assign(65536, 0);
    std::vector<const Map *> cts;
    for (Map *m : maps)
        if (m->role == ROLE_CT4 || m->role == ROLE_CT6) {
            cts.push_back(m);
            if (m->policy_lxc >= 0)
                img->ct_local[m->policy_lxc] = 1;
        }
    const Map *lbsvc = nullptr, *lbrnat = nullptr, *lb6svc = nullptr, *lb6rnat = nullptr;
    for (Map *m : maps) {
        if (m->role == ROLE_LB4_SVC)
            lbsvc = m;
        else if (m->role == ROLE_LB4_RNAT)
            lbrnat = m;
        else if (m->role == ROLE_LB6_SVC)
            lb6svc = m;
        else if (m->role == ROLE_LB6_RNAT)
            lb6rnat = m;
    }
    img->lb_ct = (lbsvc && !lbsvc->kv.empty()) || (lbrnat && !lbrnat->kv.empty());
    img->lb6_ct = (lb6svc && !lb6svc->kv.empty()) || (lb6rnat && !lb6rnat->kv.empty());
    if (groups & GROUP_LB) {
        build_lb(lbsvc, lbrnat, img);
        build_lb6(lb6svc, lb6rnat, img);
    }
    if (groups & GROUP_CT)
        build_ct(cts, img);
    const Map *ipc = nullptr, *lxc = nullptr, *pf4fix = nullptr,
              *pf4dyn = nullptr, *pf6fix = nullptr, *pf6dyn = nullptr;
    std::map<int, Map *> pols;
    for (Map *m : maps) {
        switch (m->role) {
        case ROLE_IPCACHE: ipc = m; break;
        case ROLE_LXC: lxc = m; break;
        case ROLE_PF4_FIX: pf4fix = m; break;
        case ROLE_PF4_DYN: pf4dyn = m; break;
        case ROLE_PF6_FIX: pf6fix = m; break;
        case ROLE_PF6_DYN: pf6dyn = m; break;
        case ROLE_POLICY: pols[m->policy_lxc] = m; break;
        default: break;
        }
    }

    const Map *ipc6m = (groups & GROUP_IPCACHE6) ? ipc : nullptr;
    if (!(groups & GROUP_IPCACHE4))
        ipc = nullptr;
    if (!(groups & GROUP_PREFILTER))
        pf4fix = pf4dyn = pf6fix = pf6dyn = nullptr;
    if (!(groups & GROUP_ENDPOINTS)) {
        lxc = nullptr;
        pols.clear();
    }
    if (ipc) {
        std::vector<Pfx4> pfx;
        ipcache_v4(ipc, &pfx, &img->lbl_ovf);
        img->n_prefix4 = (uint32_t)pfx.size();
        if (!pfx.empty()) {
            const size_t n_ovf = img->lbl_ovf.size();
            bool trie = opt.lpm4 != LPM4_DIR24_8;
            if (trie && !build_l4trie(pfx, &img->lbl_ovf, &img->l4d, &img->l4c,
                                      &img->l4l)) {
                img->l4d.clear();
                img->l4c.clear();
                img->l4l.clear();
                img->lbl_ovf.resize(n_ovf);
                trie = false;
            }
            if (trie) {
                img->lpm4_layout = LPM4_TRIE;
            } else {
                build_dir24_8(pfx, &img->tbl24, &img->tbl8);
                img->lpm4_layout = LPM4_DIR24_8;
            }
        }
    }

    if (ipc6m) {
        std::vector<Pfx6> pfx;
        ipcache_v6(ipc6m, &pfx);
        build_lpm6(pfx, &img->ipc6);
    }

    if (pf6fix && pf6fix->ksz == 20) {
        std::vector<Pfx6> pfx;
        prefilter_v6(pf6fix, true, &pfx);
        build_lpm6(pfx, &img->pf6_fix);
        bool all128 = !pfx.empty();
        for (const Pfx6 &p : pfx)
            all128 &= p.plen == 128;
        if (all128) {
            bloom_size(&img->pf6_bloom, 2 * pfx.size(), PF_BLOOM_MAX_WORDS);
            for (const Pfx6 &p : pfx)
                bloom_add(&img->pf6_bloom, pf6_bloom_hash(p.w[0], p.w[1], p.w[2], p.w[3]));
        }
    }
    if (pf6dyn && pf6dyn->ksz == 20) {
        std::vector<Pfx6> pfx;
        prefilter_v6(pf6dyn, false, &pfx);
        build_lpm6(pfx, &img->pf6_dyn);
    }
    if (pf4dyn && pf4dyn->ksz == 8) {
        std::vector<Pfx4> pfx;
        for (const auto &kv : pf4dyn->kv) {
            const uint8_t *k = (const uint8_t *)kv.first.data();
            uint32_t P, a;
            memcpy(&P, k, 4);
            memcpy(&a, k + 4, 4);
            pfx.push_back({bswap(a), (uint8_t)P, 1u});
        }
        img->n_pf_dyn = (uint32_t)pfx.size();
        if (!pfx.empty())
            build_dir24_8(pfx, &img->pf_tbl24, &img->pf_tbl8);
    }
    if (pf4fix && pf4fix->ksz == 8) {
        std::vector<uint32_t> addrs;
        for (const auto &kv : pf4fix->kv) {
            const uint8_t *k = (const uint8_t *)kv.first.data();
            uint32_t P, a;
            memcpy(&P, k, 4);
            memcpy(&a, k + 4, 4);
            if (P != 32)
                continue;
            if (a == 0)
                img->pf_fix_zero = 1;
            else
                addrs.push_back(a);
        }
        img->n_pf_fix = (uint32_t)addrs.size() + img->pf_fix_zero;
        if (!addrs.empty()) {
            bloom_size(&img->pf_bloom, 2 * addrs.size(), PF_BLOOM_MAX_WORDS);
            for (uint32_t a : addrs)
                bloom_add(&img->pf_bloom, pf_bloom_hash(a));
            uint32_t nb = pow2_at_least(addrs.size());
            img->pf_fix.assign((size_t)nb * PF_SLOTS, 0);
            img->pf_fix_mask = nb - 1;
            for (uint32_t a : addrs) {
                uint32_t b = hash32(a, nb - 1);
                for (;;) {
                    uint32_t *bk = &img->pf_fix[(size_t)b * PF_SLOTS];
                    int s = 0;
                    while (s < PF_SLOTS && bk[s])
                        s++;
                    if (s < PF_SLOTS) {
                        bk[s] = a;
                        break;
                    }
                    b = (b + 1) & (nb - 1);
                }
            }
        }
    }
// ... 113 lines not shown
```

cilium_amd/csrc/flatten.hpp:

```cpp
#pragma once
#include <cstdint>
#include <map>
#include <string>
#include <unordered_map>
#include <utility>
#include <vector>

#include "layout.h"
#include "maps.hpp"

namespace cfc {

struct PolLoc {
    uint32_t base = 0, mask = 0, present = 0;
};

enum Lpm4Layout { LPM4_AUTO = 0, LPM4_DIR24_8 = 1, LPM4_TRIE = 2 };

struct BuildOpts {
    int lpm4 = LPM4_AUTO;
};

struct Pfx6 {
    uint32_t w[4];
    uint8_t plen;
    uint32_t label;
};
struct Lpm6Host {
    std::vector<L6Slot> slots;
    std::vector<uint4> slots64;
    std::vector<uint64_t> bloom;
    std::vector<uint32_t> lens;
    uint32_t def_label = 0;
    uint32_t n = 0;
    uint32_t groups = 0;
    uint64_t bytes() const
    {
        return sizeof(L6Slot) * slots.size() + 16ull * slots64.size() + 8ull * bloom.size() +
               4ull * lens.size();
    }
};
constexpr int64_t L6_S64 = (int64_t)1 << 40;
void build_lpm6(const std::vector<Pfx6> &pfx, Lpm6Host *out);
bool ipcache_v6_entry(const std::string &nk, const std::string &val, Pfx6 *p);
int64_t lpm6_find_slot(const Lpm6Host &t, const Pfx6 &p);
uint32_t lpm6_lookup_host(const Lpm6Host &t, const uint32_t w[4]);

struct HostImage {
    uint64_t ct_min4 = 0, ct_min6 = 0;
    std::vector<uint32_t> tbl24, tbl8, lbl_ovf;
    std::vector<uint32_t> l4d, l4c;
    std::vector<uint64_t> l4l;
    int lpm4_layout = 0;
    uint32_t n_prefix4 = 0;
    std::vector<uint32_t> pf_tbl24, pf_tbl8;
    uint32_t n_pf_dyn = 0;
    std::vector<uint32_t> pf_fix;
    uint32_t pf_fix_mask = 0, pf_fix_zero = 0, n_pf_fix = 0;
    std::vector<uint32_t> pf_bloom;
    std::vector<uint32_t> pf6_bloom;
    std::vector<LxcSlot> lxc4;
    uint32_t lxc4_mask = 0, n_eps = 0;
    std::vector<PolSlot> pol;
    std::vector<uint32_t> pol_bloom;
    std::unordered_map<int, PolLoc> pol_loc;
    Lpm6Host ipc6, pf6_fix, pf6_dyn;
    std::vector<Lxc6Slot> lxc6;
    uint32_t lxc6_mask = 0, n_eps6 = 0;
    std::map<uint16_t, uint32_t> nat4;
    std::map<uint16_t, uint4> nat6;
    std::vector<std::pair<Map *, std::string>> ctr_owner;
    std::vector<Ct4Slot> ct4;
    std::vector<Ct6Slot> ct6;
    std::vector<CtTimer> ct4_tm, ct6_tm;
    uint32_t ct4_mask = 0, ct4_probe = 0, ct6_mask = 0, ct6_probe = 0;
    uint32_t n_ct4 = 0, n_ct6 = 0;
    uint32_t n_nat46 = 0;
    std::vector<uint8_t> ct_local;
    std::vector<uint4> lb4;
    uint32_t lb4_mask = 0, n_lb4 = 0;
    std::vector<uint2> rnat4;
    std::vector<uint4> ct4_lb;
    bool lb_ct = false;
    std::vector<uint4> lb6;
    uint32_t lb6_mask = 0, n_lb6 = 0;
    std::vector<uint4> rnat6;
    std::vector<uint4> ct6_lb;
    bool lb6_ct = false;
    uint64_t device_bytes() const;
};

uint64_t ct_map_key(int family, uint32_t owner, int any);
bool ct_slot_of(const Map *m, const std::string &key, Ct4Slot *s4, Ct6Slot *s6);
CtTimer ct_timer_of(const std::string &val);
uint4 ct_lb_of(const std::string &val);

enum : unsigned {
    GROUP_IPCACHE4 = 1,
    GROUP_PREFILTER = 2,
    GROUP_ENDPOINTS = 4,
    GROUP_CT = 8,
    GROUP_IPCACHE6 = 16,
    GROUP_LB = 32,
    GROUP_ALL = 63,
};
void build_image(const std::vector<Map *> &maps, const BuildOpts &opt,
                 HostImage *img, unsigned groups = GROUP_ALL);

struct Pfx4 {
    uint32_t addr;
    uint8_t plen;
    uint32_t leaf;
};
void build_dir24_8(std::vector<Pfx4> pfx, std::vector<uint32_t> *tbl24,
                   std::vector<uint32_t> *tbl8);
bool build_l4trie(std::vector<Pfx4> pfx, std::vector<uint32_t> *ovf,
                  std::vector<uint32_t> *l4d, std::vector<uint32_t> *l4c,
                  std::vector<uint64_t> *l4l);

}
```

cilium_amd/csrc/kern_common.hpp:

```cpp
#pragma once
#include "classify.hpp"

namespace cfc {

namespace {

constexpr uint32_t HOST_ID = 1, WORLD_ID = 2, CLUSTER_ID = 3, HEALTH_ID = 4;
constexpr int DROP_INVALID_SIP = -132, DROP_POLICY = -133,
              DROP_CT_UNKNOWN_PROTO = -137, DROP_MISSED_TAIL_CALL = -140,
              DROP_NO_SERVICE = -158, DROP_INVALID = -134;
constexpr int TC_ACT_OK = 0, TC_ACT_SHOT = 2, TC_ACT_REDIRECT = 7;
constexpr int XDP_DROP = 1, XDP_PASS = 2;
constexpr int METRIC_INGRESS = 1, METRIC_EGRESS = 2;
constexpr uint32_t NONE = 0xFFFFFFFFu;
constexpr uint64_t COUNT_PER_BLOCK = 63 * BLOCK;

__device__ __forceinline__ uint32_t notify_word(int mode, int ver,
                                                bool dest_stage,
                                                uint32_t dest_lxc,
                                                uint32_t ep_lxc)
{
    if (ver >= 0 || ver == CFC_DROP_PREFILTER || ver == CFC_VERDICT_PUNT)
        return 0;
    if (mode == CFC_MODE_EGRESS)
// ... 36 lines not shown
#define CFC_WG_PER_CU 2
#endif
constexpr int WAVES_PER_SIMD = 4 * CFC_WG_PER_CU;
constexpr size_t LDS_PER_WG = LDS_BYTES_MAX / CFC_WG_PER_CU;

template <class T>
__device__ __forceinline__ T ld_nt(const T *p)
{
    return __builtin_nontemporal_load(p);
}
template <class T>
__device__ __forceinline__ void st_nt(T v, T *p)
{
    __builtin_nontemporal_store(v, p);
}
template <class T>
__device__ __forceinline__ T ldo_nt(const T *base, uint32_t off)
{
    return __builtin_nontemporal_load(
        reinterpret_cast<const T *>(reinterpret_cast<const char *>(base) + off));
}
template <class T>
__device__ __forceinline__ void sto_nt(T v, T *base, uint32_t off)
{
    __builtin_nontemporal_store(v, reinterpret_cast<T *>(reinterpret_cast<char *>(base) + off));
}
template <class T>
__device__ __forceinline__ void sto(T v, T *base, uint32_t off)
{
    *reinterpret_cast<T *>(reinterpret_cast<char *>(base) + off) = v;
}

typedef uint32_t u32x4 __attribute__((ext_vector_type(4)));
__device__ __forceinline__ uint4 ld_nt4(const uint32_t *p)
{
    const u32x4 v = __builtin_nontemporal_load(reinterpret_cast<const u32x4 *>(p));
    return make_uint4(v.x, v.y, v.z, v.w);
}

__device__ __forceinline__ uint4 ld16(const void *p)
{
    return *reinterpret_cast<const uint4 *>(p);
}

__device__ __forceinline__ uint4 ldt16(const void *base, uint32_t off)
{
    const __amdgpu_buffer_rsrc_t r = __builtin_amdgcn_make_buffer_rsrc(
        const_cast<void *>(base), (short)0, 0x7FFFFFFF, 0x00020000);
    const u32x4 v = __builtin_amdgcn_raw_buffer_load_b128(r, off, 0, 0);
    return make_uint4(v.x, v.y, v.z, v.w);
}

extern __shared__ uint4 cfc_smem[];

struct Lds {
    bool lxc, pfb, polb;
    uint32_t lxc_off;
    uint32_t pfb_off, polb_off;
    uint32_t pfb_mask, polb_mask;
};

__device__ __forceinline__ unsigned long long *lds_met()
{
    return reinterpret_cast<unsigned long long *>(cfc_smem);
}
__device__ __forceinline__ uint32_t lds_word(uint32_t off)
{
    return reinterpret_cast<const uint32_t *>(cfc_smem)[off];
}

__device__ __forceinline__ uint32_t l4_leaf(const DevTables &T, uint32_t e)
{
    return (e & LPM_INDIRECT) ? T.lbl_ovf[e & LPM_PAYLOAD] : e;
}
__device__ __forceinline__ uint32_t l4_list_leaf(const DevTables &T, uint32_t hi)
{
    const uint32_t l = hi & (LL_INDIRECT | LL_PAYLOAD);
    return (l & LL_INDIRECT) ? T.lbl_ovf[l & LL_PAYLOAD] : l;
}
__device__ __forceinline__ uint32_t l4_lookup(const DevTables &T, uint32_t a,
                                              uint4 d)
{
    const uint32_t e1 = (d.z >> 16) | (d.w << 16);
    if (l4_inline_match(a, d.y))
        return l4_list_leaf(T, (d.y >> 21) | (d.z << 11));
    if (l4_inline_match(a, e1))
        return l4_list_leaf(T, d.w >> 5);
    uint32_t e = d.x;
    uint32_t shift = 16;
    while (e & L4_PTR) {
        const uint32_t cnt = (e >> 24) & 127, off = e & L4_OFF;
        if (cnt == 0) {
            shift -= 8;
            e = T.l4c[off + ((a >> shift) & 255)];
            continue;
        }
        for (uint32_t i = 0; i < cnt; i += 2) {
            const uint4 v = ldt16(T.l4l, (off + i) * 8u);
            const bool m0 = l4_match(a, v.x, v.y);
            if (m0 || l4_match(a, v.z, v.w))
                return l4_list_leaf(T, m0 ? v.y : v.w);
        }
        return 0;
    }
    return l4_leaf(T, e);
}

__device__ __forceinline__ uint4 lxc_slot(const DevTables &T, const Lds &S,
                                          uint32_t s)
{
    return S.lxc ? cfc_smem[S.lxc_off + s] : ld16(T.lxc4 + s);
}
__device__ __forceinline__ uint4 lxc_resolve(const DevTables &T, const Lds &S,
                                             uint32_t addr, uint32_t s, uint4 v)
{
    for (;;) {
        if (!(v.w & LXC_VALID))
            return make_uint4(0, 0, 0, 0);
        if (v.x == addr)
            return v;
        s = (s + 1) & T.lxc4_mask;
        v = lxc_slot(T, S, s);
    }
}

__device__ __forceinline__ bool pf_resolve(const DevTables &T, uint32_t addr,
                                           uint32_t b, uint4 v)
{
    for (;;) {
        if (v.x == addr || v.y == addr || v.z == addr || v.w == addr)
            return true;
        if (!v.x || !v.y || !v.z || !v.w)
            return false;
        b = (b + 1) & T.pf_fix_mask;
        v = ldt16(T.pf_fix, b * 16u);
    }
}

__device__ __forceinline__ bool bloom_maybe(uint32_t off, uint32_t mask,
                                            uint32_t h)
{
    const uint32_t b = bloom_bits(h);
    return (lds_word(off + ((uint32_t)h & mask)) & b) == b;
}

__device__ __forceinline__ uint64_t pkey(uint32_t id, uint32_t dport,
                                         uint32_t proto, uint32_t egress)
{
    return (uint64_t)id | ((uint64_t)dport << 32) | ((uint64_t)proto << 48) |
           ((uint64_t)egress << 56);
}

__device__ __forceinline__ bool ct_new_dport(uint32_t proto, uint32_t ports,
                                             uint32_t *dport)
{
    const bool tu = (proto == 6) | (proto == 17);
    *dport = tu ? ports >> 16 : ((ports & 0xFF) == 8 ? 8u : 0u);
    return tu | (proto == 1);
}

constexpr int CT_NEW = 0, CT_ESTABLISHED = 1, CT_REPLY = 2, CT_RELATED = 3;
constexpr int CT_EGRESS = 0, CT_INGRESS = 1, CT_SERVICE = 2;
constexpr uint32_t CTO_DONE = 4u, CTO_CREATE = 8u;

struct CtProbe {
    uint32_t z1, z2, w1, w2, td, ts;
};
template <bool V6>
__device__ __forceinline__ CtProbe ct_probe(uint32_t proto, uint32_t pt,
                                            int dir, uint32_t owner)
{
    CtProbe k;
    uint32_t fl = dir == CT_INGRESS ? 0u : dir == CT_SERVICE ? 4u : 1u;
    if (proto == 6 || proto == 17) {
        k.td = pt & 0xFFFF;
        k.ts = pt >> 16;
    } else {
// ... 621 lines not shown
```

cilium_amd/csrc/layout.h:

```cpp
#pragma once
#include <stdint.h>
#include <hip/hip_runtime.h>

namespace cfc {

constexpr uint32_t LPM_GROUP = 0x80000000u;
constexpr uint32_t LPM_INDIRECT = 0x40000000u;
constexpr uint32_t LPM_PAYLOAD = 0x3FFFFFFFu;

constexpr uint32_t EMPTY = 0xFFFFFFFFu;

constexpr uint32_t L4_PTR = 0x80000000u;
constexpr uint32_t L4_OFF = 0xFFFFFFu;
constexpr uint32_t L4_LIST_MAX = 16;
constexpr uint32_t L4_INLINE = 2;
constexpr uint32_t LL_INDIRECT = 1u << 26;
constexpr uint32_t LL_PAYLOAD = (1u << 26) - 1;
__host__ __device__ inline bool l4_match(uint32_t a, uint32_t addr, uint32_t hi)
{
    const uint32_t len = hi >> 27;
    const uint32_t m = len ? 0xFFFFFFFFu << (32 - len) : 0xFFFFFFFFu;
    return (a & m) == addr;
}
__host__ __device__ inline uint64_t l4_inline_entry(uint32_t addr, uint32_t len,
                                                    uint32_t leaf27)
{
    return (uint64_t)(addr & 0xFFFFu) | (uint64_t)(len - 16) << 16 |
           (uint64_t)leaf27 << 21;
}
__host__ __device__ inline bool l4_inline_match(uint32_t a, uint32_t e_lo32)
{
    const uint32_t l = (e_lo32 >> 16) & 31;
    const uint32_t m = (0xFFFFu << (16 - l)) & 0xFFFFu;
    return l != 0 && ((a ^ e_lo32) & m) == 0;
}

constexpr uint64_t POL_EMPTY = ~0ull;
struct alignas(16) PolSlot {
    uint64_t key;
    uint16_t proxy_port;
    uint16_t pad;
    uint32_t ctr;
};

constexpr uint32_t LXC_HOST = 1u << 16;
constexpr uint32_t LXC_HAS_POLICY = 1u << 17;
constexpr uint32_t LXC_IFINDEX = 1u << 18;
constexpr uint32_t LXC_CT_LOCAL = 1u << 19;
constexpr uint32_t LXC_HAS6 = 1u << 20;
constexpr uint32_t LXC_VALID = 1u << 31;
struct alignas(16) LxcSlot {
    uint32_t addr;
    uint32_t pol_base;
    uint32_t pol_mask;
    uint32_t info;
};

constexpr int PF_SLOTS = 4;

__host__ __device__ inline uint32_t fmix32(uint32_t h)
{
    h ^= h >> 16;
    h *= 0x85ebca6bu;
    h ^= h >> 13;
    h *= 0xc2b2ae35u;
    h ^= h >> 16;
    return h;
}
__host__ __device__ inline uint32_t hash32(uint32_t k, uint32_t mask)
{
    uint64_t x = (uint64_t)k * 0x9E3779B97F4A7C15ull;
    return (uint32_t)(x >> 32) & mask;
}
__host__ __device__ inline uint32_t pol_key_pre(uint32_t lo, uint32_t hi)
{
    return fmix32(lo * 0x9E3779B1u ^ hi);
}
__host__ __device__ inline uint32_t pol_slot(uint32_t pre, uint32_t mask)
{
    return pre & mask;
}

__host__ __device__ inline uint32_t bloom_bits(uint32_t h)
{
    return (1u << ((h >> 17) & 31)) | (1u << ((h >> 22) & 31)) | (1u << (h >> 27));
}
__host__ __device__ inline uint32_t pol_bloom_salt(uint32_t base)
{
    return (base + 1u) * 0x9E3779B1u;
}
__host__ __device__ inline uint32_t pol_bloom_hash(uint32_t salt, uint32_t pre)
{
    return pre ^ (salt >> 16) ^ (pre >> 19);
}
__host__ __device__ inline uint32_t pf_bloom_hash(uint32_t addr)
{
    return fmix32(addr ^ 0x5bd1e995u);
}
constexpr uint32_t POL_BLOOM_MAX_WORDS = 8192;
constexpr uint32_t PF_BLOOM_MAX_WORDS = 8192;
constexpr uint32_t LXC_LDS_MAX_SLOTS = 512;

constexpr uint32_t L6_GROUP_FIRST = 1u << 16;
constexpr uint32_t L6_GROUP_MAX = 4;
struct alignas(16) L6Slot {
    uint32_t w[4];
    uint32_t label;
    uint32_t len;
    uint32_t pad[2];
};
struct Lpm6 {
    const L6Slot *slots;
    const uint4 *slots64;
    const uint64_t *bloom;
    const uint32_t *lens;
    uint32_t mask;
    uint32_t mask64;
// ... 58 lines not shown
{
    uint32_t h = ct_hash4(d[0], d[1], d[2], d[3]);
    h = fmix32(h ^ s[0]);
    h = fmix32(h ^ s[1]);
    h = fmix32(h ^ s[2]);
    h = fmix32(h ^ s[3]);
    return ct_hash4(h, z, w, 0x7f4a7c15u);
}
__host__ __device__ inline uint32_t ct_home4(uint32_t x, uint32_t y, uint32_t z, uint32_t w)
{
    const uint32_t lo = x < y ? x : y, hi = x < y ? y : x;
    const uint32_t pa = z & 0xFFFFu, pb = z >> 16;
    const uint32_t zs = (pa < pb ? pa : pb) | (pa < pb ? pb : pa) << 16;
    return ct_hash4(lo, hi, zs, w & ~0x100u);
}
__host__ __device__ inline uint32_t ct_home6(const uint32_t d[4], const uint32_t s[4],
                                             uint32_t z, uint32_t w)
{
    const uint32_t hd = ct_hash4(d[0], d[1], d[2], d[3]), hs = ct_hash4(s[0], s[1], s[2], s[3]);
    const uint32_t pa = z & 0xFFFFu, pb = z >> 16;
    const uint32_t zs = (pa < pb ? pa : pb) | (pa < pb ? pb : pa) << 16;
    return ct_hash4(hd < hs ? hd : hs, hd < hs ? hs : hd, zs, (w & ~0x100u) ^ 0x7f4a7c15u);
}
struct alignas(16) Ct4Slot {
    uint32_t x, y, z, w;
};
struct alignas(16) CtTimer {
    uint32_t last_rx, last_tx;
    uint32_t flags;
    uint32_t lifetime;
};
constexpr uint32_t CTT_NON_SYN = 1u << 18;
constexpr uint32_t CTT_NAT46 = 1u << 19;
struct CtInfo {
    uint32_t sec;
    uint32_t y;
};
constexpr uint32_t CTI_UPDATED = 1u << 16, CTI_CREATED = 2u << 16, CTI_DELETED = 4u << 16;
constexpr uint32_t CTI_FRESH = 8u << 16;
constexpr uint32_t CT_CLAIM = 0xE000u;
struct alignas(16) Ct6Slot {
    uint32_t d[4], s[4], z, w, pad[2];
};
struct alignas(64) CtState {
    CtTimer tm;
    uint64_t acct[4];
    CtInfo info;
    uint32_t pad[2];
};
static_assert(sizeof(CtState) == 64, "one line per CT slot");

__host__ __device__ inline uint32_t lb4_hash(uint32_t addr, uint32_t ps)
{
    return fmix32(fmix32(addr ^ 0x85ebca6bu) ^ ps);
}
constexpr uint32_t IPV4_LOOPBACK = 0x1FFFF50Au;
__host__ __device__ inline uint32_t lb6_hash(uint32_t a0, uint32_t a1, uint32_t a2, uint32_t a3,
                                             uint32_t ps)
{
    return l6_hash(a0, a1, a2, a3, ps ^ 0x6b43a9b5u);
}

struct DevTables {
    const uint4 *l4d;
    const uint32_t *l4c;
    const uint64_t *l4l;
    const uint32_t *tbl24;
    const uint32_t *tbl8;
    const uint32_t *lbl_ovf;
    const uint32_t *pf_tbl24;
    const uint32_t *pf_tbl8;
    const uint32_t *pf_fix;
    const LxcSlot *lxc4;
    const PolSlot *pol;
    const uint32_t *pf_bloom;
    const uint32_t *pol_bloom;
    uint32_t pf_fix_mask;
    uint32_t pf_fix_zero;
    uint32_t lxc4_mask;
    uint32_t n_ctr;
    uint32_t pf_bloom_words;
    uint32_t pol_bloom_words;
    uint32_t lxc4_lds;
    Lpm6 ipc6;
    Lpm6 pf6_fix;
    Lpm6 pf6_dyn;
    const uint32_t *pf6_bloom;
    uint32_t pf6_bloom_words;
    const Lxc6Slot *lxc6;
    uint32_t lxc6_mask;
    uint32_t lxc6_lds;
    const Ct4Slot *ct4;
    const Ct6Slot *ct6;
    CtState *ct_st;
    uint32_t *ct_sum;
    uint32_t ct4_mask, ct4_probe;
    uint32_t ct6_mask, ct6_probe;
    uint32_t ct6_acct_base;
    uint32_t now;
    uint32_t host_ifindex;
    uint32_t nat46;
    uint32_t id_cover;
    uint32_t v4_cluster_range;
    uint32_t v4_cluster_mask;
    uint32_t router6[4];
    const uint4 *lb4;
    uint32_t lb4_mask;
    const uint2 *rnat4;
    const uint4 *ct4_lb;
    const uint4 *lb6;
    uint32_t lb6_mask;
    const uint4 *rnat6;
    const uint4 *ct6_lb;
};

constexpr int METRIC_REASONS = 256;
constexpr int METRIC_DIRS = 4;
constexpr int METRIC_U64 = METRIC_REASONS * METRIC_DIRS * 2;

}
```

cilium_amd/csrc/selftest.cpp:

```cpp
#include <cstdio>
#include <cerrno>
#include <cstring>
#include <map>
#include <random>
#include <vector>

#include "classify.hpp"
#include "flatten.hpp"
#include "maps.hpp"
#include "selfcut.hpp"
#include "ctmirror.hpp"

using namespace cfc;

template <bool V6>
struct ReplayCase {
    using F = CtFamily<V6>;
    using Rec = typename F::SyncRec;
    CtTab<typename F::Slot> T;
    Map tcp, any;
    CtMaps maps;
    int fail = 0;
    ReplayCase()
    {
// ... 217 lines not shown
static uint32_t brute(const std::vector<Pfx6> &pfx, const uint32_t w[4])
{
    int best = -1;
    uint32_t label = 0;
    for (const Pfx6 &p : pfx) {
        bool ok = true;
        for (int i = 0; i < 4 && ok; i++)
            ok = (w[i] & l6_word_mask(p.plen, i)) == p.w[i];
        if (ok && (int)p.plen > best) {
            best = p.plen;
            label = p.label;
        }
    }
    return label;
}

static void add(std::vector<Pfx6> &v, const uint32_t a[4], int len, uint32_t label)
{
    Pfx6 p;
    p.plen = (uint8_t)len;
    p.label = label;
    for (int i = 0; i < 4; i++)
        p.w[i] = a[i] & l6_word_mask(len, i);
    for (const Pfx6 &q : v)
        if (q.plen == p.plen && !memcmp(q.w, p.w, 16))
            return;
    v.push_back(p);
}

template <class R>
static int run(const char *name, const std::vector<Pfx6> &pfx, R &rng,
               int queries)
{
    Lpm6Host t;
    build_lpm6(pfx, &t);
    int bad = 0;
    for (int q = 0; q < queries; q++) {
        uint32_t w[4];
        for (int i = 0; i < 4; i++)
            w[i] = rng();
        if (!pfx.empty() && (q & 3)) {
            const Pfx6 &p = pfx[rng() % pfx.size()];
            for (int i = 0; i < 4; i++)
                w[i] = p.w[i] | (w[i] & ~l6_word_mask(p.plen, i));
        }
        const uint32_t a = lpm6_lookup_host(t, w), b = brute(pfx, w);
        if (a != b && bad++ < 5)
            printf("%s: %08x:%08x:%08x:%08x -> %u, want %u\n", name, w[0], w[1],
                   w[2], w[3], a, b);
    }
    printf("%-12s prefixes %5zu lengths %3zu groups %3u bloom %6zu slots %6zu: %s\n",
           name, pfx.size(), t.lens.size(), t.groups, t.bloom.size(), t.slots.size(),
           bad ? "FAIL" : "ok");
    return bad != 0;
}

static int clear_suffix_kats()
{
    struct { uint32_t len, w[4]; } k[] = {
        {128, {0xffffffffu, 0xffffffffu, 0xffffffffu, 0xffffffffu}},
        {127, {0xffffffffu, 0xffffffffu, 0xffffffffu, 0xfffffffeu}},
        {95, {0xffffffffu, 0xffffffffu, 0xfffffffeu, 0}},
        {1, {0x80000000u, 0, 0, 0}},
        {0, {0, 0, 0, 0}},
    };
    int bad = 0;
    for (const auto &c : k)
        for (int i = 0; i < 4; i++)
            bad += l6_word_mask(c.len, i) != c.w[i];
    printf("clear_suffix kats: %s\n", bad ? "FAIL" : "ok");
    return bad != 0;
}

static uint32_t dir24_lookup_host(const std::vector<uint32_t> &t24,
                                  const std::vector<uint32_t> &t8, uint32_t a)
{
    uint32_t e = t24[a >> 8];
    if (e & LPM_GROUP)
        e = t8[((size_t)(e & ~LPM_GROUP) << 8) | (a & 255)];
    return e;
}
static uint32_t l4_lookup_host(const std::vector<uint32_t> &d, const std::vector<uint32_t> &c,
                               const std::vector<uint64_t> &l, const std::vector<uint32_t> &ovf,
                               uint32_t a)
{
    auto list_leaf = [&](uint32_t hi) {
        const uint32_t x = hi & (LL_INDIRECT | LL_PAYLOAD);
        return (x & LL_INDIRECT) ? ovf[x & LL_PAYLOAD] : x;
    };
    const uint32_t *D = &d[4 * (a >> 16)];
    const uint32_t e1 = (D[2] >> 16) | (D[3] << 16);
    if (l4_inline_match(a, D[1]))
        return list_leaf((D[1] >> 21) | (D[2] << 11));
    if (l4_inline_match(a, e1))
        return list_leaf(D[3] >> 5);
    uint32_t e = D[0], shift = 16;
    while (e & L4_PTR) {
        const uint32_t cnt = (e >> 24) & 127, off = e & L4_OFF;
        if (cnt == 0) {
            shift -= 8;
            e = c[off + ((a >> shift) & 255)];
            continue;
        }
        for (uint32_t i = 0; i < cnt; i += 2) {
            const uint64_t u = l[off + i], v = l[off + i + 1];
            const bool m0 = l4_match(a, (uint32_t)u, (uint32_t)(u >> 32));
            if (m0 || l4_match(a, (uint32_t)v, (uint32_t)(v >> 32)))
                return list_leaf(m0 ? (uint32_t)(u >> 32) : (uint32_t)(v >> 32));
        }
        return 0;
    }
    return (e & LPM_INDIRECT) ? ovf[e & LPM_PAYLOAD] : e;
}
static int lpm4_case(const char *name, std::vector<Pfx4> pfx, std::mt19937 &gen, int nq)
{
    {
        std::map<std::pair<uint32_t, int>, Pfx4> u;
        for (Pfx4 p : pfx) {
            p.addr &= p.plen ? 0xFFFFFFFFu << (32 - p.plen) : 0u;
            u.emplace(std::make_pair(p.addr, (int)p.plen), p);
        }
        pfx.clear();
        for (auto &kv : u)
            pfx.push_back(kv.second);
    }
    std::vector<uint32_t> t24, t8, ovf, d, c;
    std::vector<uint64_t> l;
    build_dir24_8(pfx, &t24, &t8);
    const bool ok = build_l4trie(pfx, &ovf, &d, &c, &l);
    int bad = !ok;
    for (int q = 0; q < nq; q++) {
        uint32_t a = gen();
        if (!pfx.empty() && (q & 3)) {
            const Pfx4 &p = pfx[gen() % pfx.size()];
            const uint32_t m = p.plen ? 0xFFFFFFFFu << (32 - p.plen) : 0u;
            a = p.addr | (a & ~m);
        }
        uint32_t want = 0;
        int best = -1;
        for (const Pfx4 &p : pfx) {
            const uint32_t m = p.plen ? 0xFFFFFFFFu << (32 - p.plen) : 0u;
            if ((int)p.plen > best && (a & m) == p.addr)
                best = p.plen, want = p.leaf;
        }
        const uint32_t x = dir24_lookup_host(t24, t8, a), y = l4_lookup_host(d, c, l, ovf, a);
        if ((x != want || y != want) && bad++ < 5)
            printf("%s: %08x -> dir24 %u, trie %u, want %u\n", name, a, x, y, want);
    }
    printf("lpm4 %-14s prefixes %5zu chunks %5zu list %6zu: %s\n", name, pfx.size(),
           c.size() / 256, l.size(), bad ? "FAIL" : "ok");
    return bad != 0;
}
static int lpm4_tests(std::mt19937 &gen)
{
    int fail = 0;
    std::vector<Pfx4> v;
    for (int i = 0; i < 4000; i++)
        v.push_back({(uint32_t)gen(), (uint8_t)(gen() % 33),
                     (i % 9) ? 1 + (uint32_t)(gen() % 100000) : (1u << 27) + i});
    fail |= lpm4_case("random", v, gen, 40000);
    v.clear();
    for (int i = 0; i < 3000; i++)
        v.push_back({0x0A140000u | (uint32_t)(gen() & 0xFFFF), (uint8_t)(17 + gen() % 16),
                     1 + (uint32_t)i});
    v.push_back({0x0A140000u, 16, 77});
    v.push_back({0, 0, 5});
    fail |= lpm4_case("piled", v, gen, 40000);
    v.clear();
    for (int i = 0; i < 600; i++)
        v.push_back({0x0A141E00u | (uint32_t)(gen() & 0xFF), (uint8_t)(25 + gen() % 8),
                     1 + (uint32_t)i});
    for (int i = 0; i < 40; i++)
        v.push_back({0x0A140000u | (uint32_t)(gen() & 0xFFFF), (uint8_t)(17 + gen() % 16),
                     (1u << 26) + (uint32_t)i});
    fail |= lpm4_case("deep", v, gen, 40000);
    for (int n : {1, 2, 3, 15, 16, 17}) {
        v.clear();
        for (int i = 0; i < n; i++)
            v.push_back({0xC0A80000u | (uint32_t)(gen() & 0xFFFF), (uint8_t)(17 + gen() % 16),
                         100 + (uint32_t)i});
        char nm[32];
        snprintf(nm, sizeof nm, "small-%d", n);
        fail |= lpm4_case(nm, v, gen, 5000);
    }
    return fail;
}

static int map_fuzz(std::mt19937 &gen)
{
    int bad = 0;
    {
        Map m;
        m.type = MT_HASH, m.ksz = 8, m.vsz = 8, m.max_entries = 64;
        std::map<uint64_t, uint64_t> model;
        for (int it = 0; it < 200000; it++) {
            const uint64_t k = gen() % 96, v = gen();
            const int op = gen() % 4;
            if (op <= 1) {
                const uint64_t fl = gen() % 3;
                const bool has = model.count(k) != 0;
                const int want = fl == 1 && has ? -EEXIST : fl == 2 && !has ? -ENOENT
                                 : !has && model.size() >= 64 ? -E2BIG : 0;
                bad += m.update(&k, &v, fl) != want;
                if (!want)
                    model[k] = v;
            } else if (op == 2) {
                uint64_t got = 0;
                const int rc = m.lookup(&k, &got);
                bad += model.count(k) ? (rc != 0 || got != model[k]) : rc != -ENOENT;
            } else {
                bad += m.erase(&k) != (model.erase(k) ? 0 : -ENOENT);
            }
        }
        std::map<uint64_t, int> seen;
        uint64_t cur = 0, nxt = 0;
        for (int rc = m.next_key(nullptr, &nxt); !rc; rc = m.next_key(&cur, &nxt))
            seen[cur = nxt]++;
        bad += seen.size() != model.size();
        for (auto &kv : seen)
            bad += kv.second != 1 || !model.count(kv.first);
    }
    {
        Map m;
        m.type = MT_LPM_TRIE, m.ksz = 8, m.vsz = 4, m.max_entries = 48;
        std::map<std::pair<uint32_t, uint32_t>, uint32_t> model;
        auto msk = [](uint32_t a, uint32_t p) { return p ? a & (0xFFFFFFFFu << (32 - p)) : 0u; };
        for (int it = 0; it < 100000; it++) {
            const uint32_t plen = gen() % 34, a = gen() & 0xFF0F00FFu, v = gen();
            uint8_t key[8];
            const uint32_t be = __builtin_bswap32(a);
            memcpy(key, &plen, 4);
            memcpy(key + 4, &be, 4);
            const int op = gen() % 3;
            if (op == 0) {
                const auto mk = std::make_pair(plen, plen <= 32 ? msk(a, plen) : 0u);
                const int want = plen > 32 ? -EINVAL
                                 : !model.count(mk) && model.size() >= 48 ? -ENOSPC : 0;
                bad += m.update(key, &v, 0) != want;
                if (!want)
                    model[mk] = v;
            } else if (op == 1) {
                uint32_t got = 0, want = 0;
                int best = -1;
                for (auto &e : model)
                    if ((int)e.first.first > best && e.first.first <= std::min(plen, 32u) &&
                        msk(a, e.first.first) == e.first.second)
                        best = (int)e.first.first, want = e.second;
                const int rc = m.lookup(key, &got);
                bad += best < 0 ? rc != -ENOENT : (rc != 0 || got != want);
            } else if (plen <= 32) {
                bad += m.erase(key) != (model.erase(std::make_pair(plen, msk(a, plen))) ? 0
                                                                                         : -ENOENT);
            }
        }
    }
    printf("map fuzz (hash, lpm): %s\n", bad ? "FAIL" : "ok");
    return bad != 0;
}

static int hist_slot_case(const char *name, const std::vector<uint32_t> &lens)
{
    uint32_t slot = 0;
    uint64_t carries = 0, wraps = 0, packets = 0, bytes = 0;
    for (uint32_t len : lens) {
        uint32_t carry, wrap;
        HistSlot::spill(slot, len, carry, wrap);
// ... 4 lines not shown
        bytes += len;
    }
    const uint64_t pk = HistSlot::packets(slot) + HistSlot::esc_packets(carries, wraps);
    const uint64_t by = HistSlot::bytes(slot) + HistSlot::esc_bytes(carries);
    const bool ok = pk == packets && by == bytes;
    if (!ok)
        printf("hist slot %s n=%zu: packets %llu want %llu, bytes %llu want %llu\n", name,
               lens.size(), (unsigned long long)pk, (unsigned long long)packets,
               (unsigned long long)by, (unsigned long long)bytes);
    return !ok;
}
static int hist_slot_tests(std::mt19937 &gen)
{
    int bad = 0;
    const uint32_t pick[] = {0, 1, 59, 1500, 65534, 65535};
    for (size_t n : {(size_t)1, (size_t)2047, (size_t)2048, (size_t)2049, (size_t)100000}) {
        std::vector<uint32_t> v(n);
        std::fill(v.begin(), v.end(), 65535u);
        bad += hist_slot_case("max", v);
        std::fill(v.begin(), v.end(), 0u);
        bad += hist_slot_case("zero", v);
        for (size_t i = 0; i < n; i++)
            v[i] = (i & 1) ? 65535u : 0u;
        bad += hist_slot_case("alternating", v);
        for (size_t i = 0; i < n; i++)
            v[i] = gen() & 0xFFFF;
        bad += hist_slot_case("random", v);
        for (size_t i = 0; i < n; i++)
            v[i] = pick[gen() % 6];
        bad += hist_slot_case("mixed", v);
    }
    bad += ID_RANGES > 32 || id_range_of(ID_PACK_LIMIT - 1) != ID_RANGES - 1 ||
           2 * ID_RANGE != HIST_RANGE;
    printf("hist slot u32 {%u | %u}, %u ranges of %u identities     %s\n", HistSlot::PK,
           HistSlot::BY, ID_RANGES, ID_RANGE, bad ? "FAIL" : "ok");
    return bad != 0;
}

static void hash_kats()
{
    const uint32_t V[] = {0u, 0xFFFFFFFFu, 1u, 0x0100000Au, 0x9E3779B9u, 0x80000000u, 0x1010u};
    const uint32_t MASKS[] = {0u, 7u, 511u, 0xFFFFu, 0xFFFFFFFFu};
    for (uint32_t a : V) {
        printf("kat fmix32 %x %x\n", a, fmix32(a));
        printf("kat bloom_bits %x %x\n", a, bloom_bits(a));
        printf("kat pol_bloom_salt %x %x\n", a, pol_bloom_salt(a));
        printf("kat pf_bloom_hash %x %x\n", a, pf_bloom_hash(a));
        printf("kat l6_bloom_bits %x %llx\n", a, (unsigned long long)l6_bloom_bits(a));
        for (uint32_t m : MASKS) {
            printf("kat hash32 %x %x %x\n", a, m, hash32(a, m));
            printf("kat pol_slot %x %x %x\n", a, m, pol_slot(a, m));
        }
        for (uint32_t b : V) {
            printf("kat pol_key_pre %x %x %x\n", a, b, pol_key_pre(a, b));
            printf("kat pol_bloom_hash %x %x %x\n", a, b, pol_bloom_hash(a, b));
        }
    }
    for (uint32_t len : {0u, 1u, 31u, 32u, 33u, 63u, 64u, 65u, 95u, 96u, 97u, 127u, 128u})
        for (int i = 0; i < 4; i++)
            printf("kat l6_word_mask %x %x %x\n", len, (uint32_t)i, l6_word_mask(len, i));
    const uint32_t W[][4] = {{0, 0, 0, 0},
                             {0xFFFFFFFFu, 0xFFFFFFFFu, 0xFFFFFFFFu, 0xFFFFFFFFu},
                             {0x20010db8u, 0x00050000u, 0, 1},
                             {0xbeef0000u, 0, 0x00000001u, 0x016582bcu},
                             {1, 2, 3, 4}};
    for (const auto &w : W) {
        for (uint32_t tag : {0u, 1u, 64u, 65u, 128u, 0x200u, 0xFFFFFFFFu})
            printf("kat l6_hash %x %x %x %x %x %x\n", w[0], w[1], w[2], w[3], tag,
                   l6_hash(w[0], w[1], w[2], w[3], tag));
        for (uint32_t sel : {1u, 32u, 33u, 48u, 64u, 65u, 127u, 128u})
            printf("kat l6_group_hash %x %x %x %x %x %x\n", w[0], w[1], w[2], w[3], sel,
                   l6_group_hash(w, sel));
        printf("kat pf6_bloom_hash %x %x %x %x %x\n", w[0], w[1], w[2], w[3],
               pf6_bloom_hash(w[0], w[1], w[2], w[3]));
    }
}

int main(int argc, char **argv)
{
    hash_kats();
    if (argc > 1 && !strcmp(argv[1], "kat"))
        return 0;
    std::mt19937 gen(12345);
    auto rng = [&gen]() -> uint32_t { return (uint32_t)gen(); };
    int fail = 0;
    {
        const int lens[] = {32, 40, 48, 48, 48, 56, 56, 64, 64, 64, 96, 128, 128};
        std::vector<Pfx6> v;
        for (int i = 0; i < 3000; i++) {
            uint32_t a[4] = {0x20000000u | (rng() & 0x0FFFFFFFu), rng(), rng(), rng()};
            add(v, a, lens[rng() % 13], 256 + i);
        }
        fail |= run("c3-like", v, rng, 20000);
    }
    {
        std::vector<Pfx6> v;
        uint32_t base[4] = {0x20010db8u, 0x00050000u, 0, 0};
        add(v, base, 48, 1000);
        for (int n = 0; n < 40; n++) {
            uint32_t a[4] = {base[0], base[1] | (rng() & 0xFFFF), rng(), rng()};
            add(v, a, 64, 2000 + n);
            for (int k = 0; k < 30; k++) {
                uint32_t b[4] = {a[0], a[1], rng(), rng()};
                add(v, b, 128, 5000 + 100 * n + k);
            }
        }
        uint32_t z[4] = {0, 0, 0, 0};
        add(v, z, 0, 7);
        fail |= run("piled", v, rng, 20000);
    }
    {
        std::vector<Pfx6> v;
        uint32_t a[4] = {0x20010db8u, 0x12345678u, 0x9abcdef0u, 0x0fedcba9u};
        for (int len = 1; len <= 128; len++)
            add(v, a, len, (len % 7) ? 100 + len : 0);
        for (int i = 0; i < 500; i++) {
            uint32_t b[4] = {rng(), rng(), rng(), rng()};
            add(v, b, 1 + rng() % 128, (i % 5) ? 300 + i : 0);
        }
        fail |= run("all-lengths", v, rng, 20000);
    }
    {
        std::vector<Pfx6> v;
        for (int i = 0; i < 5000; i++) {
            uint32_t a[4] = {rng(), rng(), rng(), rng()};
            add(v, a, 128, 1);
        }
        fail |= run("exact128", v, rng, 20000);
        fail |= run("empty", std::vector<Pfx6>(), rng, 1000);
    }
    fail |= selfcut_tests();
    fail |= clear_suffix_kats();
    fail |= map_fuzz(gen);
    fail |= lpm4_tests(gen);
    fail |= hist_slot_tests(gen);
    fail |= ReplayCase<false>().run();
    fail |= ReplayCase<true>().run();
    return fail;
}
```

cilium_amd/datapath.py:

```python
from __future__ import annotations

import ctypes
import dataclasses

from . import _lib as L


@dataclasses.dataclass
class HeaderBatchV4:
    saddr: "torch.Tensor"
    daddr: "torch.Tensor"
    ports: "torch.Tensor"
    meta: "torch.Tensor"
    mark: "torch.Tensor | None" = None
    tcp_flags: "torch.Tensor | None" = None
    hash: "torch.Tensor | None" = None

    def __len__(self):
        return int(self.saddr.numel())

    def slice(self, a, b):
        sl = lambda x: None if x is None else x[a:b]
        return type(self)(*(sl(getattr(self, f.name))
                            for f in dataclasses.fields(self)))
# ... 389 lines not shown

    def proxy_apply(self, batch, out: Verdicts, mode=L.MODE_INGRESS, ep_lxc=0,
                    stream=None):
        v6 = isinstance(batch, HeaderBatchV6)
        st = L.ProxyStats()
        fn = self.L.cfc_proxy_apply_v6 if v6 else self.L.cfc_proxy_apply_v4
        L.check(fn(self.h, ctypes.byref(hdr_struct(batch)), ctypes.byref(out_struct(out)),
                   mode, ep_lxc, ctypes.byref(st), self._stream(stream)), "proxy apply")
        return {k: getattr(st, k) for k, _ in L.ProxyStats._fields_}

    def set_clock(self, now):
        L.check(self.L.cfc_set_clock(self.h, int(now) & 0xFFFFFFFF), "clock")
        self.clock = int(now) & 0xFFFFFFFF

    clock = 0

    def ct_gc(self, fd=-1, time=0, remove_expired=True, valid_ips=None,
              match_ips=None, stream=None):
        def ips(lst):
            if lst is None:
                return None, 0
            lst = [bytes(a) for a in lst]
            arr = (L.Ip * max(len(lst), 1))()
            for i, a in enumerate(lst):
                arr[i].family = 4 if len(a) == 4 else 6
                arr[i].addr[:len(a)] = list(a)
            return arr, len(lst)
        va, nv = ips(valid_ips)
        ma, nm = ips(match_ips)
        f = L.GcFilter()
        f.flags = ((L.GC_REMOVE_EXPIRED if remove_expired else 0) |
                   (L.GC_VALID_IPS if va is not None else 0) |
                   (L.GC_MATCH_IPS if ma is not None else 0))
        f.time = int(time) & 0xFFFFFFFF
        f.valid_ips = ctypes.cast(va, ctypes.c_void_p) if va is not None else None
        f.n_valid = nv
        f.match_ips = ctypes.cast(ma, ctypes.c_void_p) if ma is not None else None
        f.n_match = nm
        st = L.GcStats()
        L.check(self.L.cfc_ct_gc(self.h, int(fd), ctypes.byref(f), ctypes.byref(st),
                                 self._stream(stream)), "ct gc")
        return {k: getattr(st, k) for k, _ in L.GcStats._fields_}

    def counters_sync(self, stream=None):
        L.check(self.L.cfc_counters_sync(self.h, self._stream(stream)),
                "counters sync")

    def counters_clear(self, stream=None):
        L.check(self.L.cfc_counters_clear(self.h, self._stream(stream)),
                "counters clear")

    def counters_export(self, t, stream=None):
        L.check(self.L.cfc_counters_export(self.h, _ptr(t), t.numel(),
                                           self._stream(stream)), "export")

    def counters_import(self, t, stream=None):
        L.check(self.L.cfc_counters_import(self.h, _ptr(t), t.numel(),
                                           self._stream(stream)), "import")

    def counters_device(self):
        p, n = ctypes.c_void_p(), ctypes.c_uint64()
        L.check(self.L.cfc_counters_device(self.h, ctypes.byref(p),
                                           ctypes.byref(n)), "counters device")
        return p.value, n.value

    def identity_counters(self):
        import numpy as np
        n = ctypes.c_uint64()
        L.check(self.L.cfc_identity_counters(self.h, None, 0, ctypes.byref(n)),
                "identity counters")
        rows = (L.IdentityCount * max(n.value, 1))()
        L.check(self.L.cfc_identity_counters(self.h, rows, n.value, ctypes.byref(n)),
                "identity counters")
        return np.array([(r.identity, r.dir, r.fwd_packets, r.fwd_bytes,
                          r.drop_packets, r.drop_bytes) for r in rows[:n.value]],
                        np.uint64).reshape(-1, 6)

    def stats(self):
        st = L.Stats()
        L.check(self.L.cfc_get_stats(self.h, ctypes.byref(st)), "stats")
        return {f: getattr(st, f) for f, _ in L.Stats._fields_ if f != "pad0"}


def host_only():
    return Datapath(L.CFC_DEVICE_NONE)


def errno_name(e: OSError):
    import errno
    return errno.errorcode.get(e.errno, str(e.errno))


__all__ = ["Datapath", "HeaderBatchV4", "HeaderBatchV6", "Verdicts", "pack_v4",
           "pack_v6", "pack", "host_only", "errno_name"]
```

include/cfc.h:

```cpp
#ifndef CFC_H
#define CFC_H

#include <stddef.h>
#include <stdint.h>

#ifdef __cplusplus
extern "C" {
#endif

#define CFC_ABI_VERSION 13

typedef struct cfc_ctx cfc_ctx;

#define CFC_DEVICE_NONE (-1)
int cfc_open(int device, cfc_ctx **out);
void cfc_close(cfc_ctx *ctx);
int cfc_abi_version(void);

#define CFC_MAP_TYPE_HASH 1
#define CFC_MAP_TYPE_PERCPU_HASH 5
#define CFC_MAP_TYPE_LRU_HASH 9
#define CFC_MAP_TYPE_LPM_TRIE 11

#define CFC_ANY 0
#define CFC_NOEXIST 1
#define CFC_EXIST 2

int cfc_map_open(cfc_ctx *ctx, const char *path, uint32_t map_type,
                 uint32_t key_size, uint32_t value_size,
                 uint32_t max_entries, uint32_t flags, int *fd,
                 int *created);
int cfc_map_close(cfc_ctx *ctx, int fd);
int cfc_map_update(cfc_ctx *ctx, int fd, const void *key, const void *value,
                   uint64_t flags);
int cfc_map_update_batch(cfc_ctx *ctx, int fd, const void *keys,
                         const void *values, uint64_t count, uint64_t flags);
int cfc_map_lookup(cfc_ctx *ctx, int fd, const void *key, void *value);
int cfc_map_delete(cfc_ctx *ctx, int fd, const void *key);
int cfc_map_get_next_key(cfc_ctx *ctx, int fd, const void *key,
                         void *next_key);
int cfc_map_dump(cfc_ctx *ctx, int fd, void *keys, void *values, uint64_t cap,
                 uint64_t *n);
int cfc_num_possible_cpus(void);

int cfc_endpoint_config(cfc_ctx *ctx, uint16_t lxc_id, uint32_t seclabel);

typedef struct {
    uint32_t ipv4_cluster_range;
    uint32_t ipv4_cluster_mask;
    uint8_t router_ip6[16];
    uint32_t host_ifindex;
} cfc_node_config;
int cfc_set_node_config(cfc_ctx *ctx, const cfc_node_config *cfg);
int cfc_get_node_config(cfc_ctx *ctx, cfc_node_config *cfg);

int cfc_set_clock(cfc_ctx *ctx, uint32_t now_sec);

int cfc_commit(cfc_ctx *ctx, void *stream);

#define CFC_OPT_LPM4 1
#define CFC_LPM4_AUTO 0
#define CFC_LPM4_DIR24_8 1
#define CFC_LPM4_TRIE 2
#define CFC_OPT_TIMING 2
#define CFC_OPT_CT_APPLY 3
#define CFC_CT_APPLY_DEVICE 0
#define CFC_CT_APPLY_HOST 1
#define CFC_OPT_CT_EVICT 4
int cfc_set_option(cfc_ctx *ctx, int option, int64_t value);

#define CFC_MODE_INGRESS 0
#define CFC_MODE_EGRESS 1
#define CFC_MODE_XDP 2
#define CFC_MODE_FULL 3

#define CFC_HF_FRAG 0x100u
#define CFC_HF_TCP_CLOSE 0x200u

typedef struct {
    const uint32_t *saddr;
    const uint32_t *daddr;
    const uint32_t *ports;
    const uint32_t *meta;
    const uint32_t *mark;
    const uint8_t *tcp_flags;
    uint64_t n;
    const uint32_t *hash;
} cfc_hdr_v4;

#define CFC_HF_EXTHDR 0x400u
typedef struct {
    const uint8_t *saddr;
    const uint8_t *daddr;
    const uint32_t *ports;
    const uint32_t *meta;
    const uint32_t *mark;
    const uint8_t *tcp_flags;
    uint64_t n;
    const uint32_t *hash;
} cfc_hdr_v6;

#define CFC_DROP_PREFILTER (-1)
#define CFC_VERDICT_PUNT (-2)
#define CFC_CT_RES_MASK 0x3u
#define CFC_CT_DONE 0x4u
#define CFC_CT_CREATE 0x8u
#define CFC_NT_NETDEV 1u
#define CFC_NT_EGRESS 2u
#define CFC_NT_POLICY 3u
#define CFC_NT_TRACE 4u
#define CFC_NT_NATLEN 0x01000000u
typedef struct {
    int32_t *verdict;
    uint32_t *identity;
    uint8_t *action;
    uint8_t *ct;
    uint32_t *notify;
    uint32_t *pkt_saddr;
    uint32_t *pkt_daddr;
    uint32_t *pkt_ports;
} cfc_out;

int cfc_classify_v4(cfc_ctx *ctx, const cfc_hdr_v4 *in, const cfc_out *out,
                    int mode, uint16_t ep_lxc, void *stream);
int cfc_classify_v6(cfc_ctx *ctx, const cfc_hdr_v6 *in, const cfc_out *out,
                    int mode, uint16_t ep_lxc, void *stream);

int cfc_ct_apply_v4(cfc_ctx *ctx, const cfc_hdr_v4 *in, const cfc_out *out,
                    int mode, uint16_t ep_lxc, void *stream);
int cfc_ct_apply_v6(cfc_ctx *ctx, const cfc_hdr_v6 *in, const cfc_out *out,
                    int mode, uint16_t ep_lxc, void *stream);

#define CFC_GC_REMOVE_EXPIRED 1u
#define CFC_GC_VALID_IPS 2u
#define CFC_GC_MATCH_IPS 4u
typedef struct {
    uint8_t family;
    uint8_t pad[3];
    uint8_t addr[16];
} cfc_ip;
typedef struct {
    uint32_t flags;
    uint32_t time;
    const cfc_ip *valid_ips;
    uint32_t n_valid;
    uint32_t pad0;
    const cfc_ip *match_ips;
    uint32_t n_match;
    uint32_t pad1;
} cfc_ct_gc_filter;
typedef struct {
// ... 73 lines not shown
    uint64_t created;
    uint64_t updated;
    uint64_t failed;
} cfc_proxy_stats;

int cfc_proxy_entries_v4(cfc_ctx *ctx, const cfc_hdr_v4 *in, const cfc_out *out,
                         int mode, uint16_t ep_lxc, cfc_proxy4_entry *records,
                         uint64_t *hdr_index, uint64_t cap, uint64_t *count,
                         void *stream);
int cfc_proxy_entries_v6(cfc_ctx *ctx, const cfc_hdr_v6 *in, const cfc_out *out,
                         int mode, uint16_t ep_lxc, cfc_proxy6_entry *records,
                         uint64_t *hdr_index, uint64_t cap, uint64_t *count,
                         void *stream);
int cfc_proxy_apply_v4(cfc_ctx *ctx, const cfc_hdr_v4 *in, const cfc_out *out,
                       int mode, uint16_t ep_lxc, cfc_proxy_stats *st,
                       void *stream);
int cfc_proxy_apply_v6(cfc_ctx *ctx, const cfc_hdr_v6 *in, const cfc_out *out,
                       int mode, uint16_t ep_lxc, cfc_proxy_stats *st,
                       void *stream);

int cfc_counters_device(cfc_ctx *ctx, uint64_t **dev_ptr, uint64_t *n_u64);
int cfc_counters_sync(cfc_ctx *ctx, void *stream);
int cfc_counters_clear(cfc_ctx *ctx, void *stream);
int cfc_counters_export(cfc_ctx *ctx, uint64_t *dst, uint64_t n_u64,
                        void *stream);
int cfc_counters_import(cfc_ctx *ctx, const uint64_t *src, uint64_t n_u64,
                        void *stream);

#define CFC_IDENTITY_OUT_OF_RANGE 0xFFFFFFFFu
typedef struct {
    uint32_t identity;
    uint8_t dir;
    uint8_t pad[3];
    uint64_t fwd_packets, fwd_bytes;
    uint64_t drop_packets, drop_bytes;
} cfc_identity_count;
int cfc_identity_counters(cfc_ctx *ctx, cfc_identity_count *rows, uint64_t cap,
                          uint64_t *n);

typedef struct {
    uint64_t epoch;
    uint64_t device_bytes;
    uint32_t ipcache_v4_prefixes;
    uint32_t lpm4_tbl8_groups;
    uint32_t policy_entries;
    uint32_t endpoints;
    uint32_t prefilter_v4_fix;
    uint32_t prefilter_v4_dyn;
    uint32_t lpm4_layout;
    uint32_t lpm4_kib;
    uint32_t ipcache_v6_prefixes;
    uint32_t lpm6_lengths;
    uint32_t lpm6_groups;
    uint32_t lpm6_kib;
    uint32_t endpoints_v6;
    uint32_t prefilter_v6_fix;
    uint32_t prefilter_v6_dyn;
    uint32_t ct4_entries;
    uint32_t ct6_entries;
    uint32_t ct_apply_device;
    uint32_t ct_apply_host;
    uint32_t ct_slots;
    uint32_t ct_grown;
    uint64_t ct_order_changed;
    uint64_t nat_hops;
    uint64_t ct_evicted;
    uint64_t svc_ordered;
    uint64_t ct_apply_sparse;
    uint64_t ct_self_segments;
} cfc_stats;
int cfc_get_stats(cfc_ctx *ctx, cfc_stats *st);
const char *cfc_strerror(int err);

typedef struct {
    uint64_t launches;
    double classify_ms;
    double count_ms;
    uint64_t launches_v6;
    double classify_v6_ms;
    double count_v6_ms;
} cfc_timing;
int cfc_timing_collect(cfc_ctx *ctx, cfc_timing *out);

#ifdef __cplusplus
}
#endif
#endif
```

Baseline: 55930.

## Make LPM4 trie directory width configurable and auto-select 16-18 bits

The IPv4 LPM trie directory was fixed at 16 bits. It now supports 16, 17 or 18 bits, with sub-chunk widths adapting to the remaining bits. By default the width is chosen automatically: it is widened while more than a tenth of the prefixes would miss the inline directory slots and the table stays within a 3 MiB budget. The fast kernel is templated on the directory width so the shift stays a compile-time constant. The aim is to cut pointer-chasing into chunk levels and list scans on 100k-prefix ipcaches, at the cost of larger directory tables (more cache footprint), more kernel instantiations, and a new option plus a stats API.

```diff
diff --git a/cilium_amd/_lib.py b/cilium_amd/_lib.py
--- a/cilium_amd/_lib.py
+++ b/cilium_amd/_lib.py
@@ -9,6 +9,7 @@
 HF_FRAG, HF_TCP_CLOSE, HF_EXTHDR = 0x100, 0x200, 0x400
 DROP_PREFILTER, VERDICT_PUNT = -1, -2
 OPT_LPM4, OPT_TIMING, OPT_CT_APPLY, OPT_CT_EVICT = 1, 2, 3, 4
+OPT_LPM4_DIR_BITS = 5
 CT_APPLY_DEVICE, CT_APPLY_HOST = 0, 1
 LPM4_AUTO, LPM4_DIR24_8, LPM4_TRIE = 0, 1, 2
 
@@ -26,7 +27,7 @@
     "cfc_set_clock", "cfc_monitor_events_v4", "cfc_monitor_events_v6",
     "cfc_map_dump", "cfc_ct_gc",
     "cfc_proxy_entries_v4", "cfc_proxy_entries_v6",
-    "cfc_proxy_apply_v4", "cfc_proxy_apply_v6",
+    "cfc_proxy_apply_v4", "cfc_proxy_apply_v6", "cfc_lpm4_dir_stats",
 )
 CT_NEW, CT_ESTABLISHED, CT_REPLY, CT_RELATED = 0, 1, 2, 3
 CT_RES_MASK, CT_DONE, CT_CREATE = 0x3, 0x4, 0x8
@@ -133,6 +134,11 @@
                 ("failed", ctypes.c_uint64)]
 
 
+class Lpm4DirStat(ctypes.Structure):
+    _fields_ = [("prefixes", ctypes.c_uint64), ("unresolved", ctypes.c_uint64),
+                ("bytes", ctypes.c_uint64)]
+
+
 class Timing(ctypes.Structure):
     _fields_ = [("launches", ctypes.c_uint64), ("classify_ms", ctypes.c_double),
                 ("count_ms", ctypes.c_double), ("launches_v6", ctypes.c_uint64),
@@ -196,6 +202,8 @@
     L.cfc_identity_counters.argtypes = [vp, vp, u64, ctypes.POINTER(u64)]
     L.cfc_set_option.argtypes = [vp, i32, ctypes.c_int64]
     L.cfc_timing_collect.argtypes = [vp, ctypes.POINTER(Timing)]
+    if hasattr(L, "cfc_lpm4_dir_stats"):
+        L.cfc_lpm4_dir_stats.argtypes = [vp, ctypes.POINTER(Lpm4DirStat), pint]
     L.cfc_strerror.argtypes = [i32]
     L.cfc_strerror.restype = ctypes.c_char_p
     _lib = L
diff --git a/cilium_amd/csrc/cfc_api.cpp b/cilium_amd/csrc/cfc_api.cpp
--- a/cilium_amd/csrc/cfc_api.cpp
+++ b/cilium_amd/csrc/cfc_api.cpp
@@ -35,6 +35,7 @@
 struct GIpc {
     DevBuf tbl24, tbl8, ovf, l4d, l4c, l4l;
     int layout = 0;
+    uint32_t l4_shift = 16;
     uint32_t n_prefix4 = 0, tbl8_groups = 0, lpm4_kib = 0;
     uint64_t bytes = 0;
 };
@@ -248,6 +249,7 @@
         sig[g] = 1469598103934665603ull + (uint64_t)g;
     auto mix = [&](int g, uint64_t v) { sig[g] = (sig[g] ^ v) * 1099511628211ull; };
     mix(0, (uint64_t)c->opts.lpm4);
+    mix(0, (uint64_t)c->opts.lpm4_dir_bits);
     mix(2, c->seclabel_gen);
     for (auto &kv : c->maps) {
         const Map *m = kv.second.get();
@@ -599,6 +601,8 @@
         (*rc = upload_vec(g->l4c, img.l4c, s)) || (*rc = upload_vec(g->l4l, img.l4l, s)))
         return nullptr;
     g->layout = img.lpm4_layout;
+    if (img.l4_dir_bits)
+        g->l4_shift = 32u - (uint32_t)img.l4_dir_bits;
     g->n_prefix4 = img.n_prefix4;
     g->tbl8_groups = (uint32_t)(img.tbl8.size() / 256);
     g->lpm4_kib = (uint32_t)((4ull * (img.l4d.size() + img.l4c.size() + img.tbl24.size() +
@@ -793,6 +797,7 @@
     const GCt &C = *E.ct;
     const GLb &B = *E.lb;
     T.l4d = (const uint4 *)I.l4d.p;
+    T.l4_shift = I.l4_shift;
     T.l4c = (const uint32_t *)I.l4c.p;
     T.l4l = (const uint64_t *)I.l4l.p;
     T.tbl24 = (const uint32_t *)I.tbl24.p;
@@ -1340,6 +1345,11 @@
             return -EINVAL;
         c->opts.lpm4 = (int)value;
         return 0;
+    case CFC_OPT_LPM4_DIR_BITS:
+        if (value != 0 && (value < L4_DIR_BITS_MIN || value > L4_DIR_BITS_MAX))
+            return -EINVAL;
+        c->opts.lpm4_dir_bits = (int)value;
+        return 0;
     case CFC_OPT_TIMING:
         if (value != 0 && value != 1)
             return -EINVAL;
@@ -1360,6 +1370,32 @@
     default:
         return -EINVAL;
     }
+}
+
+int cfc_lpm4_dir_stats(cfc_ctx *c, cfc_lpm4_dir_stat st[3], int *auto_bits)
+{
+    if (!c || !st)
+        return -EINVAL;
+    std::lock_guard<std::recursive_mutex> g(c->mu);
+    std::vector<Pfx4> pfx;
+    std::vector<uint32_t> ovf, d, ch;
+    std::vector<uint64_t> l;
+    for (auto &kv : c->maps)
+        if (kv.second->role == ROLE_IPCACHE)
+            ipcache_v4_prefixes(kv.second.get(), &pfx, &ovf);
+    int a = l4_auto_dir_bits(pfx);
+    for (int i = 2; i >= 0; i--) {
+        const int D = L4_DIR_BITS_MIN + i;
+        st[i].prefixes = pfx.size();
+        st[i].unresolved = l4_unresolved(pfx, D);
+        build_l4trie(pfx, &ovf, &d, &ch, &l, D);
+        st[i].bytes = 4ull * (d.size() + ch.size()) + 8ull * l.size();
+        if (a == D && D > L4_DIR_BITS_MIN && st[i].bytes > L4_AUTO_BUDGET)
+            a--;
+    }
+    if (auto_bits)
+        *auto_bits = a;
+    return 0;
 }
 
 int cfc_timing_collect(cfc_ctx *c, cfc_timing *out)
diff --git a/cilium_amd/csrc/classify.hip b/cilium_amd/csrc/classify.hip
--- a/cilium_amd/csrc/classify.hip
+++ b/cilium_amd/csrc/classify.hip
@@ -154,7 +154,7 @@
 #if CFC_EXP == 1
             h.l4d = make_uint4(h.lh & 0xFFFF, 0, 0, 0);
 #else
-            h.l4d = ldt16(T.l4d, (h.lh >> 16) * 16u);
+            h.l4d = ldt16(T.l4d, (h.lh >> T.l4_shift) * 16u);
 #endif
         else if (T.tbl24)
             h.e24 = T.tbl24[h.lh >> 8];
@@ -540,13 +540,14 @@
     }
 }
 
-template <int MODE, int U, bool CT, bool NT, bool OPT, bool LB, bool FAST>
+template <int MODE, int U, bool CT, bool NT, bool OPT, bool LB, int FAST>
 __global__ __launch_bounds__(BLOCK, WAVES_PER_SIMD) void k_classify_v4(
     DevTables T, LdsPlan L, cfc_hdr_v4 in, cfc_out out, EgressArgs E,
     CountArgs C, uint64_t per_block, LbIn LI)
 {
     if (FAST) {
         T.tbl24 = T.tbl8 = T.pf_tbl24 = T.pf_tbl8 = nullptr;
+        T.l4_shift = 32 - FAST;
         __builtin_assume(T.l4d != nullptr);
         __builtin_assume(T.lxc4 != nullptr);
         if (MODE == CFC_MODE_XDP || MODE == CFC_MODE_FULL)
@@ -1510,15 +1511,22 @@
 {
     const LdsPlan L = lds_plan(T);
     const bool opt = in.mark || in.tcp_flags || out.action || (CT && out.ct);
-    const bool fast = fast_shape(T, MODE, L);
-    auto kern = opt ? (fast ? k_classify_v4<MODE, CFC_UNROLL, CT, NT, true, false, true>
-                            : k_classify_v4<MODE, CFC_UNROLL, CT, NT, true, false, false>)
-                    : (fast ? k_classify_v4<MODE, CFC_UNROLL, CT, NT, false, false, true>
-                            : k_classify_v4<MODE, CFC_UNROLL, CT, NT, false, false, false>);
+    const int fast = fast_shape(T, MODE, L) ? 32 - (int)T.l4_shift : 0;
+    auto kern = opt ? k_classify_v4<MODE, CFC_UNROLL, CT, NT, true, false, 0>
+                    : k_classify_v4<MODE, CFC_UNROLL, CT, NT, false, false, 0>;
+    if (fast == 16)
+        kern = opt ? k_classify_v4<MODE, CFC_UNROLL, CT, NT, true, false, 16>
+                   : k_classify_v4<MODE, CFC_UNROLL, CT, NT, false, false, 16>;
+    else if (fast == 17)
+        kern = opt ? k_classify_v4<MODE, CFC_UNROLL, CT, NT, true, false, 17>
+                   : k_classify_v4<MODE, CFC_UNROLL, CT, NT, false, false, 17>;
+    else if (fast == 18)
+        kern = opt ? k_classify_v4<MODE, CFC_UNROLL, CT, NT, true, false, 18>
+                   : k_classify_v4<MODE, CFC_UNROLL, CT, NT, false, false, 18>;
     const LbIn none{};
     if constexpr (CT && MODE != CFC_MODE_XDP) {
         if (lb)
-            kern = k_classify_v4<MODE, CFC_UNROLL, CT, NT, true, true, false>;
+            kern = k_classify_v4<MODE, CFC_UNROLL, CT, NT, true, true, 0>;
     }
     set_lds_limit((const void *)kern, (int)LDS_PER_WG);
     hipLaunchKernelGGL(kern, dim3(grid), dim3(BLOCK), L.bytes(), s, T, L, in,
diff --git a/cilium_amd/csrc/flatten.cpp b/cilium_amd/csrc/flatten.cpp
--- a/cilium_amd/csrc/flatten.cpp
+++ b/cilium_amd/csrc/flatten.cpp
@@ -62,6 +62,7 @@
 struct L4Trie {
     std::vector<uint32_t> *d, *c, *ovf;
     std::vector<uint64_t> *l;
+    int dbits;
     bool ok = true;
 
     uint32_t list_leaf(uint32_t leaf)
@@ -92,7 +93,7 @@
                 uint64_t e[L4_INLINE] = {0, 0};
                 for (; first < longp.size() && first < L4_INLINE; first++)
                     e[first] = l4_inline_entry(longp[first].addr, longp[first].plen,
-                                               list_leaf(longp[first].leaf));
+                                               list_leaf(longp[first].leaf), 32 - dbits);
                 dir[1] = (uint32_t)e[0];
                 dir[2] = (uint32_t)(e[0] >> 32) | (uint32_t)(e[1] << 16);
                 dir[3] = (uint32_t)(e[1] >> 16);
@@ -109,17 +110,18 @@
                 ok = false;
             return L4_PTR | (uint32_t)(l->size() - off) << 24 | (uint32_t)(off & L4_OFF);
         }
-        const int nl = lvl + 8;
+        const uint32_t bits = l4_chunk_bits(32 - lvl), n = 1u << bits;
+        const int nl = lvl + (int)bits;
         const uint32_t sh = 32 - nl;
         const size_t off = c->size();
-        c->resize(off + 256, 0);
+        c->resize(off + n, 0);
         uint32_t defs[256];
-        std::fill(defs, defs + 256, def);
-        std::vector<std::vector<Pfx4>> sub(256);
+        std::fill(defs, defs + n, def);
+        std::vector<std::vector<Pfx4>> sub(n);
         std::stable_sort(longp.begin(), longp.end(),
                          [](const Pfx4 &a, const Pfx4 &b) { return a.plen < b.plen; });
         for (const Pfx4 &p : longp) {
-            const uint32_t j = (p.addr >> sh) & 255;
+            const uint32_t j = (p.addr >> sh) & (n - 1);
             if (p.plen <= nl) {
                 const uint32_t span = 1u << (nl - p.plen);
                 std::fill(defs + (j & ~(span - 1)), defs + (j & ~(span - 1)) + span, p.leaf);
@@ -127,7 +129,7 @@
                 sub[j].push_back(p);
             }
         }
-        for (uint32_t j = 0; j < 256; j++) {
+        for (uint32_t j = 0; j < n; j++) {
             const uint32_t e = node(sub[j], base | (j << sh), nl, defs[j]);
             (*c)[off + j] = e;
         }
@@ -141,30 +143,57 @@
 
 bool build_l4trie(std::vector<Pfx4> pfx, std::vector<uint32_t> *ovf,
                   std::vector<uint32_t> *l4d, std::vector<uint32_t> *l4c,
-                  std::vector<uint64_t> *l4l)
-{
+                  std::vector<uint64_t> *l4l, int dir_bits)
+{
+    const int D = dir_bits;
     std::stable_sort(pfx.begin(), pfx.end(),
                      [](const Pfx4 &a, const Pfx4 &b) { return a.plen < b.plen; });
-    l4d->assign(4u << 16, 0);
+    l4d->assign((size_t)4 << D, 0);
     l4c->clear();
     l4l->clear();
     for (const Pfx4 &p : pfx) {
-        if (p.plen > 16)
+        if (p.plen > D)
             break;
-        const uint32_t start = p.plen ? (p.addr >> 16) & ~((1u << (16 - p.plen)) - 1) : 0;
-        for (uint32_t j = start; j < start + (1u << (16 - p.plen)); j++)
-            (*l4d)[4 * j] = p.leaf;
-    }
-    std::map<uint32_t, std::vector<Pfx4>> by16;
+        const uint32_t start = p.plen ? (p.addr >> (32 - D)) & ~((1u << (D - p.plen)) - 1) : 0;
+        for (uint32_t j = start; j < start + (1u << (D - p.plen)); j++)
+            (*l4d)[4 * (size_t)j] = p.leaf;
+    }
+    std::map<uint32_t, std::vector<Pfx4>> byd;
     for (const Pfx4 &p : pfx)
-        if (p.plen > 16)
-            by16[p.addr >> 16].push_back(p);
-    L4Trie b{l4d, l4c, ovf, l4l};
-    for (auto &g : by16) {
-        uint32_t *dir = l4d->data() + 4 * g.first;
-        dir[0] = b.node(g.second, g.first << 16, 16, dir[0], dir);
+        if (p.plen > D)
+            byd[p.addr >> (32 - D)].push_back(p);
+    L4Trie b{l4d, l4c, ovf, l4l, D};
+    for (auto &g : byd) {
+        uint32_t *dir = l4d->data() + 4 * (size_t)g.first;
+        dir[0] = b.node(g.second, g.first << (32 - D), D, dir[0], dir);
     }
     return b.ok;
+}
+
+uint64_t l4_unresolved(const std::vector<Pfx4> &pfx, int dir_bits)
+{
+    std::vector<uint32_t> idx;
+    for (const Pfx4 &p : pfx)
+        if (p.plen > dir_bits)
+            idx.push_back(p.addr >> (32 - dir_bits));
+    std::sort(idx.begin(), idx.end());
+    uint64_t un = 0;
+    for (size_t i = 0, j; i < idx.size(); i = j) {
+        for (j = i; j < idx.size() && idx[j] == idx[i];)
+            j++;
+        un += j - i > L4_INLINE ? j - i - L4_INLINE : 0;
+    }
+    return un;
+}
+
+int l4_auto_dir_bits(const std::vector<Pfx4> &pfx)
+{
+    int D = L4_DIR_BITS_MIN;
+    for (; D < L4_DIR_BITS_MAX && (32ull << D) <= L4_AUTO_BUDGET; D++)
+        if (l4_unresolved(pfx, D) * L4_AUTO_SHARE_DEN < pfx.size() * L4_AUTO_SHARE_NUM ||
+            pfx.empty())
+            break;
+    return D;
 }
 
 namespace {
@@ -355,6 +384,11 @@
     for (const auto &b : best)
         out->push_back({b.first.first, (uint8_t)b.first.second,
                         leaf_for(b.second.second, ovf)});
+}
+
+void ipcache_v4_prefixes(const Map *m, std::vector<Pfx4> *out, std::vector<uint32_t> *ovf)
+{
+    ipcache_v4(m, out, ovf);
 }
 
 bool ipcache_v6_entry(const std::string &nk, const std::string &val, Pfx6 *p)
@@ -778,15 +812,25 @@
         if (!pfx.empty()) {
             const size_t n_ovf = img->lbl_ovf.size();
             bool trie = opt.lpm4 != LPM4_DIR24_8;
-            if (trie && !build_l4trie(pfx, &img->lbl_ovf, &img->l4d, &img->l4c,
-                                      &img->l4l)) {
+            for (int D = 0; D < 3; D++)
+                img->l4_unresolved[D] = l4_unresolved(pfx, L4_DIR_BITS_MIN + D);
+            int D = opt.lpm4_dir_bits ? opt.lpm4_dir_bits : l4_auto_dir_bits(pfx);
+            for (; trie; D--) {
+                img->lbl_ovf.resize(n_ovf);
+                trie = build_l4trie(pfx, &img->lbl_ovf, &img->l4d, &img->l4c, &img->l4l, D);
+                const uint64_t bytes = 4ull * (img->l4d.size() + img->l4c.size()) +
+                                       8ull * img->l4l.size();
+                if (opt.lpm4_dir_bits || D == L4_DIR_BITS_MIN || bytes <= L4_AUTO_BUDGET)
+                    break;
+            }
+            if (!trie) {
                 img->l4d.clear();
                 img->l4c.clear();
                 img->l4l.clear();
                 img->lbl_ovf.resize(n_ovf);
-                trie = false;
             }
             if (trie) {
+                img->l4_dir_bits = D;
                 img->lpm4_layout = LPM4_TRIE;
             } else {
                 build_dir24_8(pfx, &img->tbl24, &img->tbl8);
diff --git a/cilium_amd/csrc/flatten.hpp b/cilium_amd/csrc/flatten.hpp
--- a/cilium_amd/csrc/flatten.hpp
+++ b/cilium_amd/csrc/flatten.hpp
@@ -17,8 +17,13 @@
 
 enum Lpm4Layout { LPM4_AUTO = 0, LPM4_DIR24_8 = 1, LPM4_TRIE = 2 };
 
+constexpr int L4_DIR_BITS_MIN = 16, L4_DIR_BITS_MAX = 18;
+constexpr uint64_t L4_AUTO_SHARE_NUM = 1, L4_AUTO_SHARE_DEN = 10;
+constexpr uint64_t L4_AUTO_BUDGET = 3u << 20;
+
 struct BuildOpts {
     int lpm4 = LPM4_AUTO;
+    int lpm4_dir_bits = 0;
 };
 
 struct Pfx6 {
@@ -51,6 +56,8 @@
     std::vector<uint32_t> tbl24, tbl8, lbl_ovf;
     std::vector<uint32_t> l4d, l4c;
     std::vector<uint64_t> l4l;
+    int l4_dir_bits = 0;
+    uint64_t l4_unresolved[3] = {0, 0, 0};
     int lpm4_layout = 0;
     uint32_t n_prefix4 = 0;
     std::vector<uint32_t> pf_tbl24, pf_tbl8;
@@ -116,6 +123,9 @@
                    std::vector<uint32_t> *tbl8);
 bool build_l4trie(std::vector<Pfx4> pfx, std::vector<uint32_t> *ovf,
                   std::vector<uint32_t> *l4d, std::vector<uint32_t> *l4c,
-                  std::vector<uint64_t> *l4l);
+                  std::vector<uint64_t> *l4l, int dir_bits = L4_DIR_BITS_MIN);
+uint64_t l4_unresolved(const std::vector<Pfx4> &pfx, int dir_bits);
+int l4_auto_dir_bits(const std::vector<Pfx4> &pfx);
+void ipcache_v4_prefixes(const Map *m, std::vector<Pfx4> *out, std::vector<uint32_t> *ovf);
 
 }
diff --git a/cilium_amd/csrc/kern_common.hpp b/cilium_amd/csrc/kern_common.hpp
--- a/cilium_amd/csrc/kern_common.hpp
+++ b/cilium_amd/csrc/kern_common.hpp
@@ -142,17 +142,18 @@
                                               uint4 d)
 {
     const uint32_t e1 = (d.z >> 16) | (d.w << 16);
-    if (l4_inline_match(a, d.y))
+    uint32_t shift = T.l4_shift;
+    if (l4_inline_match(a, d.y, shift))
         return l4_list_leaf(T, (d.y >> 21) | (d.z << 11));
-    if (l4_inline_match(a, e1))
+    if (l4_inline_match(a, e1, shift))
         return l4_list_leaf(T, d.w >> 5);
     uint32_t e = d.x;
-    uint32_t shift = 16;
     while (e & L4_PTR) {
         const uint32_t cnt = (e >> 24) & 127, off = e & L4_OFF;
         if (cnt == 0) {
-            shift -= 8;
-            e = T.l4c[off + ((a >> shift) & 255)];
+            const uint32_t bits = l4_chunk_bits(shift);
+            shift -= bits;
+            e = T.l4c[off + ((a >> shift) & ((1u << bits) - 1))];
             continue;
         }
         for (uint32_t i = 0; i < cnt; i += 2) {
diff --git a/cilium_amd/csrc/layout.h b/cilium_amd/csrc/layout.h
--- a/cilium_amd/csrc/layout.h
+++ b/cilium_amd/csrc/layout.h
@@ -23,16 +23,20 @@
     return (a & m) == addr;
 }
 __host__ __device__ inline uint64_t l4_inline_entry(uint32_t addr, uint32_t len,
-                                                    uint32_t leaf27)
-{
-    return (uint64_t)(addr & 0xFFFFu) | (uint64_t)(len - 16) << 16 |
-           (uint64_t)leaf27 << 21;
-}
-__host__ __device__ inline bool l4_inline_match(uint32_t a, uint32_t e_lo32)
+                                                    uint32_t leaf27, uint32_t shift)
+{
+    return (uint64_t)(addr & ~(0xFFFFFFFFu << shift)) |
+           (uint64_t)(len - (32 - shift)) << 16 | (uint64_t)leaf27 << 21;
+}
+__host__ __device__ inline bool l4_inline_match(uint32_t a, uint32_t e_lo32, uint32_t shift)
 {
     const uint32_t l = (e_lo32 >> 16) & 31;
-    const uint32_t m = (0xFFFFu << (16 - l)) & 0xFFFFu;
+    const uint32_t m = (0xFFFFFFFFu << (shift - l)) & ~(0xFFFFFFFFu << shift);
     return l != 0 && ((a ^ e_lo32) & m) == 0;
+}
+__host__ __device__ inline uint32_t l4_chunk_bits(uint32_t shift)
+{
+    return shift < 8 ? shift : 8;
 }
 
 constexpr uint64_t POL_EMPTY = ~0ull;
@@ -257,6 +261,7 @@
     uint32_t pf_bloom_words;
     uint32_t pol_bloom_words;
     uint32_t lxc4_lds;
+    uint32_t l4_shift;
     Lpm6 ipc6;
     Lpm6 pf6_fix;
     Lpm6 pf6_dyn;
diff --git a/cilium_amd/csrc/selftest.cpp b/cilium_amd/csrc/selftest.cpp
--- a/cilium_amd/csrc/selftest.cpp
+++ b/cilium_amd/csrc/selftest.cpp
@@ -323,24 +323,26 @@
 }
 static uint32_t l4_lookup_host(const std::vector<uint32_t> &d, const std::vector<uint32_t> &c,
                                const std::vector<uint64_t> &l, const std::vector<uint32_t> &ovf,
-                               uint32_t a)
+                               uint32_t a, int dir_bits)
 {
     auto list_leaf = [&](uint32_t hi) {
         const uint32_t x = hi & (LL_INDIRECT | LL_PAYLOAD);
         return (x & LL_INDIRECT) ? ovf[x & LL_PAYLOAD] : x;
     };
-    const uint32_t *D = &d[4 * (a >> 16)];
+    uint32_t shift = 32u - (uint32_t)dir_bits;
+    const uint32_t *D = &d[4 * (size_t)(a >> shift)];
     const uint32_t e1 = (D[2] >> 16) | (D[3] << 16);
-    if (l4_inline_match(a, D[1]))
+    if (l4_inline_match(a, D[1], shift))
         return list_leaf((D[1] >> 21) | (D[2] << 11));
-    if (l4_inline_match(a, e1))
+    if (l4_inline_match(a, e1, shift))
         return list_leaf(D[3] >> 5);
-    uint32_t e = D[0], shift = 16;
+    uint32_t e = D[0];
     while (e & L4_PTR) {
         const uint32_t cnt = (e >> 24) & 127, off = e & L4_OFF;
         if (cnt == 0) {
-            shift -= 8;
-            e = c[off + ((a >> shift) & 255)];
+            const uint32_t bits = l4_chunk_bits(shift);
+            shift -= bits;
+            e = c.at(off + ((a >> shift) & ((1u << bits) - 1)));
             continue;
         }
         for (uint32_t i = 0; i < cnt; i += 2) {
@@ -353,7 +355,8 @@
     }
     return (e & LPM_INDIRECT) ? ovf[e & LPM_PAYLOAD] : e;
 }
-static int lpm4_case(const char *name, std::vector<Pfx4> pfx, std::mt19937 &gen, int nq)
+static int lpm4_case(const char *name, std::vector<Pfx4> pfx, std::mt19937 &gen, int nq,
+                     const std::vector<uint32_t> &probes = {})
 {
     {
         std::map<std::pair<uint32_t, int>, Pfx4> u;
@@ -365,14 +368,18 @@
         for (auto &kv : u)
             pfx.push_back(kv.second);
     }
-    std::vector<uint32_t> t24, t8, ovf, d, c;
-    std::vector<uint64_t> l;
+    std::vector<uint32_t> t24, t8, ovf[3], d[3], c[3];
+    std::vector<uint64_t> l[3];
     build_dir24_8(pfx, &t24, &t8);
-    const bool ok = build_l4trie(pfx, &ovf, &d, &c, &l);
-    int bad = !ok;
-    for (int q = 0; q < nq; q++) {
+    int bad = 0;
+    for (int D = 16; D <= 18; D++)
+        bad += !build_l4trie(pfx, &ovf[D - 16], &d[D - 16], &c[D - 16], &l[D - 16], D) ||
+               d[D - 16].size() != (size_t)4 << D;
+    for (int q = 0; q < nq + (int)probes.size(); q++) {
         uint32_t a = gen();
-        if (!pfx.empty() && (q & 3)) {
+        if (q >= nq) {
+            a = probes[q - nq];
+        } else if (!pfx.empty() && (q & 3)) {
             const Pfx4 &p = pfx[gen() % pfx.size()];
             const uint32_t m = p.plen ? 0xFFFFFFFFu << (32 - p.plen) : 0u;
             a = p.addr | (a & ~m);
@@ -384,12 +391,22 @@
             if ((int)p.plen > best && (a & m) == p.addr)
                 best = p.plen, want = p.leaf;
         }
-        const uint32_t x = dir24_lookup_host(t24, t8, a), y = l4_lookup_host(d, c, l, ovf, a);
-        if ((x != want || y != want) && bad++ < 5)
-            printf("%s: %08x -> dir24 %u, trie %u, want %u\n", name, a, x, y, want);
-    }
-    printf("lpm4 %-14s prefixes %5zu chunks %5zu list %6zu: %s\n", name, pfx.size(),
-           c.size() / 256, l.size(), bad ? "FAIL" : "ok");
+        const uint32_t x = dir24_lookup_host(t24, t8, a);
+        if (x != want && bad++ < 5)
+            printf("%s: %08x -> dir24 %u, want %u\n", name, a, x, want);
+        for (int D = 16; D <= 18; D++) {
+            const uint32_t y =
+                l4_lookup_host(d[D - 16], c[D - 16], l[D - 16], ovf[D - 16], a, D);
+            if (y != want && bad++ < 5)
+                printf("%s: %08x -> trie /%d %u, want %u\n", name, a, D, y, want);
+        }
+    }
+    for (int D = 16; D <= 18; D++)
+        printf("lpm4 %-14s /%d chunk words %6zu list %6zu unresolved %5llu -> %s\n", name, D,
+               c[D - 16].size(), l[D - 16].size(), (unsigned long long)l4_unresolved(pfx, D),
+               bad ? "FAIL" : "ok");
+    if (probes.empty())
+        printf("lpm4 %-14s prefixes %5zu: %s\n", name, pfx.size(), bad ? "FAIL" : "ok");
     return bad != 0;
 }
 static int lpm4_tests(std::mt19937 &gen)
@@ -423,6 +440,54 @@
         char nm[32];
         snprintf(nm, sizeof nm, "small-%d", n);
         fail |= lpm4_case(nm, v, gen, 5000);
+    }
+    for (int D = 16; D <= 18; D++) {
+        v.clear();
+        std::vector<uint32_t> pr;
+        const uint32_t sh = 32 - D, wide = 1u << 26;
+        const uint32_t A = 0x0A140000u;
+        v.push_back({A, (uint8_t)(D - 1), 11});
+        v.push_back({A, (uint8_t)D, 12});
+        v.push_back({A, (uint8_t)(D + 1), 13});
+        v.push_back({A + 1, 32, 14});
+        for (uint32_t o : {0u, 1u, 2u, 1u << (sh - 1), (1u << (sh - 1)) - 1, 1u << sh,
+                           (1u << sh) - 1, 2u << sh, (2u << sh) - 1, ~0u})
+            pr.push_back(A + o);
+        uint32_t k = 0;
+        for (int n : {2, 3, 14, 15}) {
+            const uint32_t N = 0x0A200000u + (k++ << sh);
+            for (int i = 0; i < n; i++) {
+                const uint32_t a = N | (uint32_t)(i + 1) << 4;
+                const uint8_t len = i == 0 ? 32 : i == n - 1 ? D + 1 : 28;
+                const uint32_t m = 0xFFFFFFFFu << (32 - len);
+                v.push_back({a & m, len,
+                             i == 0 || i == n - 1 ? wide + 100u * n + i : 100u * n + i});
+                for (uint32_t o : {0u, 1u, 15u, 16u})
+                    pr.push_back(a + o);
+            }
+            pr.push_back(N);
+            pr.push_back(N + (1u << sh) - 1);
+            pr.push_back(N + (1u << (sh - 1)));
+            pr.push_back(N + (1u << (sh - 1)) - 1);
+        }
+        const uint32_t M = 0x0A300040u;
+        for (uint32_t i = 0; i < 20; i++) {
+            const bool p31 = i % 5 == 4;
+            v.push_back({M + 3 * i - (p31 ? (3 * i) & 1 : 0), (uint8_t)(p31 ? 31 : 32),
+                         (i & 1 ? wide : 0) + 2000 + i});
+        }
+        for (uint32_t o = 0; o < 66; o++)
+            pr.push_back(M - 1 + o);
+        v.push_back({0xFFFFFF00u, 24, 31});
+        v.push_back({0xFFFFFFFFu, 32, wide + 32});
+        v.push_back({0, (uint8_t)(D + 1), 33});
+        v.push_back({1, 32, 34});
+        for (uint32_t a : {0xFFFFFFFFu, 0xFFFFFFFEu, 0xFFFFFF00u, 0xFFFFFEFFu, 0xFFFFC000u, 0u,
+                           1u, 2u, (1u << (sh - 1)) - 1, 1u << (sh - 1), 1u << sh})
+            pr.push_back(a);
+        char nm[32];
+        snprintf(nm, sizeof nm, "edges-%d", D);
+        fail |= lpm4_case(nm, v, gen, 5000, pr);
     }
     return fail;
 }
@@ -593,6 +658,8 @@
     if (argc > 1 && !strcmp(argv[1], "kat"))
         return 0;
     std::mt19937 gen(12345);
+    if (argc > 1 && !strcmp(argv[1], "lpm4"))
+        return lpm4_tests(gen);
     auto rng = [&gen]() -> uint32_t { return (uint32_t)gen(); };
     int fail = 0;
     {
diff --git a/cilium_amd/datapath.py b/cilium_amd/datapath.py
--- a/cilium_amd/datapath.py
+++ b/cilium_amd/datapath.py
@@ -495,6 +495,14 @@
         return {f: getattr(st, f) for f, _ in L.Stats._fields_ if f != "pad0"}
 
 
+    def lpm4_dir_stats(self):
+        st = (L.Lpm4DirStat * 3)()
+        auto = ctypes.c_int(0)
+        L.check(self.L.cfc_lpm4_dir_stats(self.h, st, ctypes.byref(auto)), "lpm4 dir stats")
+        return ({16 + i: {f: getattr(st[i], f) for f, _ in L.Lpm4DirStat._fields_}
+                 for i in range(3)}, auto.value)
+
+
 def host_only():
     return Datapath(L.CFC_DEVICE_NONE)
 
diff --git a/include/cfc.h b/include/cfc.h
--- a/include/cfc.h
+++ b/include/cfc.h
@@ -67,6 +67,7 @@
 #define CFC_CT_APPLY_DEVICE 0
 #define CFC_CT_APPLY_HOST 1
 #define CFC_OPT_CT_EVICT 4
+#define CFC_OPT_LPM4_DIR_BITS 5
 int cfc_set_option(cfc_ctx *ctx, int option, int64_t value);
 
 #define CFC_MODE_INGRESS 0
@@ -306,6 +307,13 @@
 } cfc_timing;
 int cfc_timing_collect(cfc_ctx *ctx, cfc_timing *out);
 
+typedef struct {
+    uint64_t prefixes;
+    uint64_t unresolved;
+    uint64_t bytes;
+} cfc_lpm4_dir_stat;
+int cfc_lpm4_dir_stats(cfc_ctx *ctx, cfc_lpm4_dir_stat st[3], int *auto_bits);
+
 #ifdef __cplusplus
 }
 #endif
```

Result: faster. 58900, median of 6 (+5.3%).
